# envoy/ksql

Measured on AMD Instinct MI355X. Metric: records/sec, windowed GROUP BY (COUNT(*) TUMBLING 5 s GROUP BY card_number HAVING > 3), higher is better.
Workload: dtype int64

## Files before the change

ksql_amd/csrc/khip_agg_c1.hip:

```cpp
#include <algorithm>
#include <cstdio>
#include <type_traits>
#include <vector>

#include "khip_part.hpp"
#include "khip_sort.hpp"

namespace khip {

constexpr int C1_TILE = 65536;
constexpr int C1_NT = 512;
constexpr int C1_CH = 8192;
template <class T>
__device__ __forceinline__ T c1_ld(const T* p) {
  return *p;
}
constexpr int C1_SEGMAX = 512;
constexpr int C1_SEGB = 7;
constexpr int C1_SEGOF = 512;
constexpr uint32_t C1_SENT = 0x80000000u;

__device__ __forceinline__ int bits_of(uint64_t v) { return v ? 64 - __clzll((long long)v) : 0; }

__device__ __forceinline__ int64_t ci_ld(const int64_t* ci, int k) {
  const uint64_t v = (uint64_t)__hip_atomic_load(&ci[k], __ATOMIC_RELAXED, __HIP_MEMORY_SCOPE_AGENT);
  const uint32_t lo = __builtin_amdgcn_readfirstlane((uint32_t)v), hi = __builtin_amdgcn_readfirstlane((uint32_t)(v >> 32));
  return (int64_t)(((uint64_t)hi << 32) | lo);
}

template <int U, int NT, class R, bool W>
__device__ __forceinline__ uint32_t stage_step_runs(const R (&rec)[U], const uint32_t (&t32)[U], const uint32_t (&bin)[U],
                                                const bool (&ok)[U], int nb, uint32_t* cnt, uint32_t* sbase, int* wsum,
                                                R* sp, uint32_t* lt32, R* __restrict__ out, uint32_t* __restrict__ outT,
                                                int64_t gs, uint32_t* lrc, uint16_t* lro) {
  const int t = threadIdx.x, lane = t & 63, wave = t >> 6;
  uint32_t rank[U];
#pragma unroll
  for (int u = 0; u < U; u++) rank[u] = ok[u] ? atomicAdd(&cnt[bin[u]], 1u) : 0u;
  lds_barrier();
  const uint32_t c = t < nb ? cnt[t] : 0u;
  uint32_t incl = c;
  for (int off = 1; off < 64; off <<= 1) {
    const uint32_t y = __shfl_up(incl, off, 64);
    if (lane >= off) incl += y;
  }
  if (lane == 63) wsum[wave] = (int)incl;
  lds_barrier();
  uint32_t before = 0, tot = 0;
#pragma unroll
  for (int k = 0; k < NT / 64; k++) {
    before += k < wave ? (uint32_t)wsum[k] : 0u;
    tot += (uint32_t)wsum[k];
  }
  if (t < nb) {
    sbase[t] = before + incl - c;
    lrc[t] = c;
    lro[t] = (uint16_t)(before + incl - c);
    cnt[t] = 0u;
  }
  lds_barrier();
#pragma unroll
  for (int u = 0; u < U; u++)
    if (ok[u]) {
      const uint32_t i = sbase[bin[u]] + rank[u];
      sp[i] = rec[u];
      if (W) lt32[i] = t32[u];
    }
  lds_barrier();
  R* o = out + gs * (int64_t)(U * NT);
  for (uint32_t j = t; j < tot; j += NT) o[j] = sp[j];
  if (W) {
    uint32_t* oT = outT + gs * (int64_t)(U * NT);
    for (uint32_t j = t; j < tot; j += NT) oT[j] = lt32[j];
  }
  return tot;
}

template <int NT, class R>
__device__ __forceinline__ void step_krange(const R* sp, uint32_t tot, uint32_t kmask, uint32_t* lkr) {
  uint32_t mn = 0xFFFFFFFFu, mx = 0u;
  for (uint32_t j = threadIdx.x; j < tot; j += NT) {
    uint64_t w;
    if constexpr (sizeof(R) == 16) w = ((const ulonglong2*)sp)[j].x;
    else w = (uint64_t)((const int64_t*)sp)[j];
    const uint32_t kr = (uint32_t)(w >> 32) & kmask;
    mn = kr < mn ? kr : mn;
    mx = kr > mx ? kr : mx;
  }
  for (int off = 32; off > 0; off >>= 1) {
    const uint32_t a = __shfl_xor(mn, off, 64), b = __shfl_xor(mx, off, 64);
    mn = a < mn ? a : mn;
    mx = b > mx ? b : mx;
  }
  if ((threadIdx.x & 63) == 0 && mx >= mn) {
    atomicMin(&lkr[0], mn);
    atomicMax(&lkr[1], mx);
  }
}

__host__ __device__ constexpr size_t run_stage_lds(int nb, int S, int rec_bytes, bool w) {
  return (size_t)nb * 8 + (size_t)S * rec_bytes + (w ? (size_t)S * 4 : 0);
}
__host__ __device__ constexpr size_t run_cnt_lds(int nb, int spt) { return (size_t)nb * spt * 6; }

template <int SPT, int NT>
__device__ __forceinline__ void flush_run_counts(const uint32_t* lrc, const uint16_t* lro, int B, int st_last, int64_t t,
                                                 int64_t nSt, uint32_t* __restrict__ rcnt, uint16_t* __restrict__ roff) {
  static_assert(SPT % 8 == 0, "whole 16-byte stores");
  for (int b = threadIdx.x; b < B; b += NT) {
    uint32_t* rc = rcnt + (int64_t)b * nSt + t * SPT;
    uint16_t* ro = roff + (int64_t)b * nSt + t * SPT;
#pragma unroll
    for (int q = 0; q < SPT / 4; q++) {
      uint32_t v[4];
#pragma unroll
      for (int k = 0; k < 4; k++) v[k] = 4 * q + k <= st_last ? lrc[(4 * q + k) * B + b] : 0u;
      *(uint4*)(rc + 4 * q) = make_uint4(v[0], v[1], v[2], v[3]);
    }
#pragma unroll
    for (int q = 0; q < SPT / 8; q++) {
      uint32_t w[4];
#pragma unroll
      for (int k = 0; k < 4; k++) {
        const int s0 = 8 * q + 2 * k;
        const uint32_t lo = s0 <= st_last ? lro[s0 * B + b] : 0u, hi = s0 + 1 <= st_last ? lro[(s0 + 1) * B + b] : 0u;
        w[k] = lo | hi << 16;
      }
      *(uint4*)(ro + 8 * q) = make_uint4(w[0], w[1], w[2], w[3]);
    }
  }
}

__device__ __forceinline__ void run_bases(const int64_t* __restrict__ keys, const int64_t* __restrict__ ts, int64_t n,
                                          const int64_t* __restrict__ stream_time, int64_t kb_in, int has_kb,
                                          int kfield, int64_t* ci, int64_t* T0, int64_t* kb) {
  const int64_t st0 = *stream_time;
  const int64_t t0 = n > 0 ? ts[0] : 0;
  *T0 = st0 >= 0 ? st0 : (t0 > 0 ? t0 : 0);
  *kb = has_kb ? kb_in : (int64_t)((uint64_t)keys[0] - (1ULL << (kfield - 1)));
  if (blockIdx.x == 0 && threadIdx.x == 0) {
    ci[CI_T0] = *T0;
    ci[CI_KBASE] = *kb;
  }
}

__device__ __forceinline__ void run_krange(const uint32_t* lkr, int kfail, int64_t kb, int64_t* ci) {
  if (lkr[1] >= lkr[0]) {
    atomicMin((long long*)&ci[CI_KMIN], (long long)((uint64_t)kb + lkr[0]));
    atomicMax((long long*)&ci[CI_KMAX], (long long)((uint64_t)kb + lkr[1]));
  }
  if (kfail) atomicOr((unsigned long long*)&ci[CI_KFAIL], 1ULL);
}

template <int U, int NT, bool WIDE, bool ST>
__global__ __launch_bounds__(NT) __attribute__((amdgpu_waves_per_eu(4))) void k_c1_scatter(
    const int64_t* __restrict__ keys, const int64_t* __restrict__ ts, const uint8_t* __restrict__ kv,
    const uint8_t* __restrict__ rv, int64_t n, int64_t nT, int log2B, uint32_t* __restrict__ rcnt,
    uint16_t* __restrict__ roff, int64_t nSt, uint64_t* __restrict__ srec, int64_t* __restrict__ tilestat,
    int64_t* __restrict__ tpart, int64_t* __restrict__ ci, const int64_t* __restrict__ st_at,
    uint32_t* __restrict__ srecT, int64_t size, int64_t adv, FastDiv fd, int64_t grace,
    const int64_t* __restrict__ stream_time, int64_t kb_in, int has_kb) {
  extern __shared__ __attribute__((aligned(16))) char smem[];
  __shared__ int wsum[NT / 64];
  __shared__ unsigned long long lc[4];
  __shared__ int lt[2][2];
  __shared__ int lfail, lkfail;
  __shared__ uint32_t lkr[2];
  constexpr int S = U * NT;
  constexpr int SPT = C1_TILE / S;
  const int B = 1 << log2B;
  const int64_t t = tile_of(blockIdx.x, nT);
  uint32_t* cnt = (uint32_t*)smem;
  uint32_t* sbase = cnt + B;
  int64_t* sp = (int64_t*)(smem + (size_t)B * 8);
  uint32_t* lt32 = (uint32_t*)(sp + S);
  uint32_t* lrc = (uint32_t*)(smem + run_stage_lds(B, S, 8, WIDE));
  uint16_t* lro = (uint16_t*)(lrc + SPT * B);
  for (int b = threadIdx.x; b < B; b += NT) cnt[b] = 0u;
  if (threadIdx.x < 4) lc[threadIdx.x] = 0;
  if (threadIdx.x < 2) {
    lt[threadIdx.x][0] = INT32_MIN;
    lt[threadIdx.x][1] = INT32_MAX;
  }
  if (threadIdx.x == 0) {
    lfail = lkfail = 0;
    lkr[0] = 0xFFFFFFFFu;
    lkr[1] = 0u;
  }
  int64_t T0, kb;
  run_bases(keys, ts, n, stream_time, kb_in, has_kb, 32, ci, &T0, &kb);
  const int shift = log2B == 0 ? 64 : 64 - log2B;
  const uint32_t bmask = (uint32_t)(B - 1);
  const int64_t base = t * C1_TILE;
  const int64_t end = base + C1_TILE < n ? base + C1_TILE : n;
  int c_acc = 0, c_nk = 0, c_nr = 0, c_bt = 0;
  uint32_t kor = 0u;
  int64_t x[U], k[U];
  auto load_step = [&](int64_t i0, int64_t (&dx)[U], int64_t (&dk)[U]) {
#pragma unroll
    for (int u = 0; u < U; u++) {
      int64_t i = i0 + (int64_t)u * NT;
      i = i < end ? i : end - 1;
      dx[u] = ts[i];
      dk[u] = keys[i];
    }
  };
  int64_t t_rmax = -1, t_min = INT64_MAX, t_bound = INT64_MAX;
  bool t_ok = true;
  auto publish = [&](int64_t, int st) {
    const int mx = lt[st & 1][0], mn = lt[st & 1][1];
    if (mx != INT32_MIN) {
      const int64_t smx = T0 + mx, smn = T0 + mn;
      t_rmax = smx > t_rmax ? smx : t_rmax;
      t_min = smn < t_min ? smn : t_min;
      const int64_t fw = first_window_start_fd(smn, size, adv, fd) + size;
      const int64_t b = grace > ((int64_t)1 << 61) ? INT64_MAX : fw + grace - 1;
      t_bound = b < t_bound ? b : t_bound;
      t_ok = t_ok && t_rmax <= b;
    }
    lt[st & 1][0] = INT32_MIN;
    lt[st & 1][1] = INT32_MAX;
  };
  lds_barrier();
  int64_t s0 = base;
  int st_last = -1;
  if (s0 < end) load_step(s0 + threadIdx.x, x, k);
  for (int st = 0; s0 < end; s0 += S, st++) {
    st_last = st;
    const int64_t i0 = s0 + threadIdx.x;
    bool ok[U];
    uint32_t bin[U], t32[U];
    int64_t rec[U];
    int tmx = INT32_MIN, tmn = INT32_MAX;
#pragma unroll
    for (int u = 0; u < U; u++) {
      const int64_t i = i0 + (int64_t)u * NT;
      ok[u] = i < end;
      const bool kok = bit_get(kv, ok[u] ? i : base), rok = bit_get(rv, ok[u] ? i : base);
      const bool valid = ok[u] && kok && rok && x[u] >= 0;
      c_nk += ok[u] && !kok;
      c_nr += ok[u] && kok && !rok;
      c_bt += ok[u] && kok && rok && x[u] < 0;
      c_acc += valid;
      const int64_t sx = ST ? st_at[ok[u] ? i : base] : x[u];
      const int64_t d = x[u] - T0;
      if (valid && (d <= (int64_t)INT32_MIN || d > (int64_t)INT32_MAX)) {
        lfail = 1;
#ifdef KHIP_TUNING
        if (ci[CI_N - 1] == 1 && (threadIdx.x & 63) == 0) printf("[c1 scatter] t %ld i %ld x %ld T0 %ld\n", (long)t, (long)i, (long)x[u], (long)T0);
#endif
      }
      if constexpr (ST) {
        const int64_t ds = sx - T0;
        if (valid && (ds <= (int64_t)INT32_MIN || ds > (int64_t)INT32_MAX)) lfail = 1;
        tmx = valid && (int)ds > tmx ? (int)ds : tmx;
      } else {
        tmx = valid && (int)d > tmx ? (int)d : tmx;
      }
      tmn = valid && (int)d < tmn ? (int)d : tmn;
      const uint64_t hk = key_hash(k[u]);
      bin[u] = stage_bin(hk, shift, bmask);
      t32[u] = valid ? (uint32_t)d : C1_SENT;
      const uint64_t kd = (uint64_t)k[u] - (uint64_t)kb;
      if (!WIDE) kor |= ok[u] ? (uint32_t)(kd >> 32) : 0u;
      rec[u] = WIDE ? (int64_t)hk : (int64_t)((kd << 32) | (uint64_t)t32[u]);
    }
    if (s0 + S < end) load_step(i0 + S, x, k);
    const uint32_t tot = stage_step_runs<U, NT, int64_t, WIDE>(rec, t32, bin, ok, B, cnt, sbase, wsum, sp, lt32,
                                                               (int64_t*)srec, srecT, t * SPT + st, lrc + st * B,
                                                               lro + st * B);
    if (!WIDE) step_krange<NT, int64_t>(sp, tot, 0xFFFFFFFFu, lkr);
    for (int off = 32; off > 0; off >>= 1) {
      const int a = __shfl_xor(tmx, off, 64), b = __shfl_xor(tmn, off, 64);
      tmx = a > tmx ? a : tmx;
      tmn = b < tmn ? b : tmn;
    }
    if ((threadIdx.x & 63) == 0 && tmx != INT32_MIN) {
      atomicMax(&lt[st & 1][0], tmx);
      atomicMin(&lt[st & 1][1], tmn);
    }
    if (threadIdx.x == 0 && st > 0) publish(s0 - S, st - 1);
  }
  flush_run_counts<SPT, NT>(lrc, lro, B, st_last, t, nSt, rcnt, roff);
  if (!WIDE && kor) lkfail = 1;
  __syncthreads();
  if (threadIdx.x == 0 && s0 > base) publish(s0 - S, st_last);
  if (!WIDE && threadIdx.x == 0) run_krange(lkr, lkfail, kb, ci);
  c_acc = wave_sum(c_acc);
  c_nk = wave_sum(c_nk);
  c_nr = wave_sum(c_nr);
  c_bt = wave_sum(c_bt);
  if ((threadIdx.x & 63) == 0) {
    if (c_acc) atomicAdd(&lc[0], (unsigned long long)c_acc);
    if (c_nk) atomicAdd(&lc[1], (unsigned long long)c_nk);
    if (c_nr) atomicAdd(&lc[2], (unsigned long long)c_nr);
    if (c_bt) atomicAdd(&lc[3], (unsigned long long)c_bt);
  }
  __syncthreads();
  if (threadIdx.x == 0) {
    int64_t* tp = tpart + t * T_NPART;
    tp[T_ACCEPTED] = (int64_t)lc[0];
    tp[T_NULL_KEY] = (int64_t)lc[1];
    tp[T_NULL_ROW] = (int64_t)lc[2];
    tp[T_BAD_TS] = (int64_t)lc[3];
    tp[T_APPLIED] = (int64_t)lc[0];
    tp[T_LATE] = 0;
    if (lfail) atomicOr((unsigned long long*)&ci[CI_TFAIL], 1ULL);
    int64_t* ts4 = tilestat + t * 4;
    ts4[0] = t_rmax;
    ts4[1] = t_min;
    ts4[2] = t_bound;
    ts4[3] = t_ok ? 1 : 0;
  }
}

__global__ __launch_bounds__(256) void k_c1_krange(const int64_t* __restrict__ keys, int64_t stride, int64_t n,
                                                   long long* __restrict__ out) {
  int64_t mx = INT64_MIN, mxn = INT64_MIN;
  for (int64_t i = blockIdx.x * (int64_t)blockDim.x + threadIdx.x; i < n; i += (int64_t)gridDim.x * blockDim.x) {
    const int64_t k = keys[i * stride];
    mx = k > mx ? k : mx;
    mxn = ~k > mxn ? ~k : mxn;
  }
  for (int off = 32; off > 0; off >>= 1) {
    const int64_t a = __shfl_xor(mx, off, 64), b = __shfl_xor(mxn, off, 64);
    mx = a > mx ? a : mx;
    mxn = b > mxn ? b : mxn;
  }
  if ((threadIdx.x & 63) == 0) {
    atomicMax(&out[0], (long long)mxn);
    atomicMax(&out[1], (long long)mx);
  }
}

__global__ __launch_bounds__(256) void k_c1_bases(const uint32_t* __restrict__ rpos, int64_t nSt, int B,
                                                  int64_t* __restrict__ bb) {
  for (int b = threadIdx.x; b <= B; b += blockDim.x) bb[b] = (int64_t)rpos[(int64_t)b * nSt];
}

__global__ __launch_bounds__(256) void k_c1_chunks(const int* __restrict__ cstart, int B, const int64_t* __restrict__ bb,
                                                   const uint32_t* __restrict__ rpos, int64_t nSt, int ch,
                                                   const int64_t* __restrict__ ci, uint32_t* __restrict__ cinfo) {
  if (ci_ld(ci, CI_GATE) == 0) return;
  const int w = blockIdx.x * blockDim.x + threadIdx.x;
  if (w >= (int)ci_ld(ci, CI_NCHUNK)) return;
  int a = 0, e = B;
  while (e - a > 1) {
    const int m = (a + e) >> 1;
    if (cstart[m] <= w) a = m;
    else e = m;
  }
  const int b = a;
  const int64_t lo = bb[b] + (int64_t)(w - cstart[b]) * ch;
  const int64_t len = bb[b + 1] - lo < ch ? bb[b + 1] - lo : ch;
  const uint32_t* rp = rpos + (int64_t)b * nSt;
  int64_t sa = 0, se = nSt;
  while (se - sa > 1) {
    const int64_t m = (sa + se) >> 1;
    if ((int64_t)rp[m] <= lo) sa = m;
    else se = m;
  }
  int64_t ta = sa, te = nSt;
  while (te - ta > 1) {
    const int64_t m = (ta + te) >> 1;
    if ((int64_t)rp[m] < lo + len) ta = m;
    else te = m;
  }
  cinfo[2 * w] = (uint32_t)sa;
  cinfo[2 * w + 1] = (uint32_t)(te - sa);
}

__device__ __forceinline__ void chunk_map(const uint32_t* __restrict__ rp, const uint16_t* __restrict__ ro,
                                          const uint32_t* __restrict__ cinfo, int w, int64_t S, int64_t lo, int len,
                                          uint32_t* map) {
  const int64_t s0 = cinfo[2 * w];
  const int R = (int)cinfo[2 * w + 1];
  for (int k = threadIdx.x; k < R; k += blockDim.x) {
    const int64_t s = s0 + k, p = (int64_t)rp[s], pe = (int64_t)rp[s + 1];
    const int64_t a = p > lo ? p : lo, e = pe < lo + len ? pe : lo + len;
    const uint32_t src = (uint32_t)(s * S + (int64_t)ro[s] + (a - p));
    for (int64_t x = a; x < e; x++) map[x - lo] = src + (uint32_t)(x - a);
  }
  __syncthreads();
}

__global__ __launch_bounds__(1024) void k_c1_check(
    const int64_t* __restrict__ tilestat, int64_t nT, int64_t size, int64_t adv, FastDiv fd, int64_t grace,
    int64_t close0, int fresh, int log2B, int log2P, int wide, int ch, int kbmax, int pbits,
    const int64_t* __restrict__ bb, int* __restrict__ cstart,
    int64_t* __restrict__ ci, int64_t* __restrict__ stream_time, int64_t* __restrict__ res,
    unsigned long long* __restrict__ ctr, unsigned long long* __restrict__ closed_ctr, unsigned long long closed_n) {
  __shared__ int64_t wmx[16];
  __shared__ int64_t red[4][16];
  __shared__ int lslow;
  __shared__ int lnch[512 + 1];
  const int lane = threadIdx.x & 63, wave = threadIdx.x >> 6;
  if (threadIdx.x == 0) lslow = 0;
  const int64_t st0 = *stream_time;
  const int64_t K = (nT + 1023) / 1024;
  const int64_t g0 = threadIdx.x * K, g1 = g0 + K < nT ? g0 + K : nT;
  int64_t m = -1;
  for (int64_t g = g0; g < g1; g++) m = tilestat[4 * g] > m ? tilestat[4 * g] : m;
  const int64_t incl = wave_incl_max(m);
  if (lane == 63) wmx[wave] = incl;
  __syncthreads();
  int64_t pre = st0;
  for (int w = 0; w < wave; w++) pre = wmx[w] > pre ? wmx[w] : pre;
  const int64_t excl = __shfl_up(incl, 1, 64);
  int64_t run = lane == 0 ? pre : (excl > pre ? excl : pre);
  int64_t gmn = INT64_MAX, gmx = -1;
  bool slow = false;
  for (int64_t g = g0; g < g1; g++) {
    const int64_t* t4 = tilestat + 4 * g;
    const int64_t mx = t4[0], mn = t4[1];
    if (mn != INT64_MAX) {
      slow |= t4[3] == 0 || run > t4[2];
      gmn = mn < gmn ? mn : gmn;
    }
    run = mx > run ? mx : run;
    gmx = mx > gmx ? mx : gmx;
  }
  if (slow) lslow = 1;
  for (int off = 32; off > 0; off >>= 1) {
    const int64_t a = __shfl_xor(gmn, off, 64), b = __shfl_xor(gmx, off, 64);
    gmn = a < gmn ? a : gmn;
    gmx = b > gmx ? b : gmx;
  }
  if (lane == 0) {
    red[0][wave] = gmn;
    red[1][wave] = gmx;
  }
  const int B = 1 << log2B;
  for (int b = threadIdx.x; b < B; b += 1024) lnch[b] = (int)((bb[b + 1] - bb[b] + ch - 1) / ch);
  __syncthreads();
  if (threadIdx.x) return;
  for (int w = 0; w < 16; w++) {
    gmn = red[0][w] < gmn ? red[0][w] : gmn;
    gmx = red[1][w] > gmx ? red[1][w] : gmx;
  }
  int acc = 0, mxc = 0;
  for (int b = 0; b < B; b++) {
    cstart[b] = acc;
    acc += lnch[b];
    mxc = lnch[b] > mxc ? lnch[b] : mxc;
  }
  cstart[B] = acc;
  const int64_t kmin = ci_ld(ci, CI_KMIN), kmax = ci_ld(ci, CI_KMAX);
  const bool tfail = ci_ld(ci, CI_TFAIL) != 0, kfail = ci_ld(ci, CI_KFAIL) != 0;
  ci[CI_KMIN] = INT64_MAX;
  ci[CI_KMAX] = INT64_MIN;
  ci[CI_TFAIL] = 0;
  ci[CI_KFAIL] = 0;
  bool ok = !lslow && !tfail && mxc <= C1_SEGMAX && (wide || kmax >= kmin);
#ifdef KHIP_TUNING
  if (ci[CI_N - 1] == 1)
    printf("[c1 check] tfail %d slow %d mxc %d kmin %ld kmax %ld gmn %ld gmx %ld T0 %ld st0 %ld nT %ld\n", (int)tfail,
           (int)lslow, mxc, (long)kmin, (long)kmax, (long)gmn, (long)gmx, (long)ci[CI_T0], (long)st0, (long)nT);
#endif
  const uint64_t krange = kmax >= kmin ? (uint64_t)kmax - (uint64_t)kmin : 0;
  const bool fits = !wide && !kfail && krange < ((1ULL << kbmax) - 1);
  const int64_t kb = ci_ld(ci, CI_KBASE);
  ci[CI_FITS] = fits ? 1 : 0;
  ci[CI_REASON] = ok && !wide && kfail ? 2 : (ok && !wide && !fits ? 1 : 0);
  ci[CI_KMINC] = kmin;
  ci[CI_KSHIFT] = (int64_t)((uint64_t)kmin - (uint64_t)kb);
  ok = ok && (wide || fits);
  int64_t lo = INT64_MAX, hi = INT64_MIN;
  if (gmx >= 0) {
    const int64_t l = gmn - size + adv;
    lo = (int64_t)fast_udiv((uint64_t)(l > 0 ? l : 0), fd);
    hi = (int64_t)fast_udiv((uint64_t)gmx, fd);
  }
  if (!fresh) {
    int64_t rlo = res[0];
    const int64_t rhi = res[1];
    if (close0 != INT64_MIN && rlo != INT64_MAX) {
      const int64_t c = close0 - size;
      const int64_t lb = c >= 0 ? (int64_t)fast_udiv((uint64_t)c, fd) + 1 : 0;
      rlo = rlo > lb ? rlo : lb;
    }
    lo = rlo < lo ? rlo : lo;
    hi = rhi > hi ? rhi : hi;
  }
  const bool none = lo > hi;
  if (none) lo = hi = 0;
  ok = ok && (uint64_t)(hi - lo) < (wide ? ((uint64_t)1 << log2P) - 1 : (pbits ? 0x7FFFFFFEull : 0xFFFFFFFEull));
  const int wbits = bits_of((uint64_t)(hi - lo)), kbits = bits_of(krange);
  ci[CI_GATE] = ok ? 1 : 0;
  if (!ok) return;
  ci[CI_WBASE] = lo;
  ci[CI_WHI] = hi - lo;
  ci[CI_WBITS] = wbits;
  ci[CI_KBITS] = kbits;
  ci[CI_KRANGE] = (int64_t)krange;
  ci[CI_ID32] = !wide && kbits + wbits + pbits <= 31 ? 1 : 0;
  ci[CI_WIDE] = wide;
  ci[CI_TMIN] = gmx >= 0 ? gmn : 0;
  ci[CI_TMAX] = gmx;
  ci[CI_NCHUNK] = acc;
  *stream_time = gmx > st0 ? gmx : st0;
  res[0] = none ? INT64_MAX : lo;
  res[1] = none ? INT64_MIN : hi;
  ctr[CTR_ADDED] = ctr[CTR_FAILED] = ctr[CTR_NEED] = 0ULL;
  if (closed_ctr) *closed_ctr = closed_n;
}

template <int U, int NT, bool WIDE>
__global__ __launch_bounds__(NT) __attribute__((amdgpu_waves_per_eu(4))) void k_c1_refine(
    const uint64_t* __restrict__ srcA, const int64_t* __restrict__ bb, const int* __restrict__ cstart, int log2B,
    int log2P, int fbits, uint64_t* __restrict__ srec, uint16_t* __restrict__ seg, const int64_t* __restrict__ ci,
    const uint32_t* __restrict__ srcAT, uint32_t* __restrict__ srecT, const uint32_t* __restrict__ rpos,
    const uint16_t* __restrict__ roff, int64_t nSt, int64_t S, const uint32_t* __restrict__ cinfo) {
  if (ci_ld(ci, CI_GATE) == 0) return;
  const int w = blockIdx.x;
  if (w >= (int)ci_ld(ci, CI_NCHUNK)) return;
  extern __shared__ __attribute__((aligned(16))) char smem[];
  __shared__ int lb, lnv;
  __shared__ int wsum[NT / 64];
  static_assert(U * NT == C1_CH, "refine chunk");
  const int F = 1 << fbits, B = 1 << log2B;
  uint32_t* cnt = (uint32_t*)smem;
  uint32_t* sbase = cnt + F;
  uint64_t* stage = (uint64_t*)(smem + (size_t)F * 8);
  for (int f = threadIdx.x; f < F; f += NT) cnt[f] = 0u;
  if (threadIdx.x == 0) lb = -1;
  __syncthreads();
  for (int b = threadIdx.x; b < B; b += NT)
    if (cstart[b] <= w && w < cstart[b + 1]) lb = b;
  __syncthreads();
  const int b = lb;
  if (b < 0) return;
  const int64_t lo = bb[b] + (int64_t)(w - cstart[b]) * C1_CH;
  const int64_t bend = bb[b + 1];
  const int len = (int)(bend - lo < C1_CH ? bend - lo : C1_CH);
  const int64_t kmin = ci_ld(ci, CI_KMINC);
  const uint64_t kshift = WIDE ? 0 : (uint64_t)ci_ld(ci, CI_KSHIFT) << 32;
  const int shift = 64 - log2P;
  const uint32_t* rp = rpos + (int64_t)b * nSt;
  const uint16_t* ro = roff + (int64_t)b * nSt;
  chunk_map(rp, ro, cinfo, w, S, lo, len, (uint32_t*)stage);
  uint64_t r[U];
  uint32_t f[U], rank[U], t32[U];
#pragma unroll
  for (int u = 0; u < U; u++) {
    const int j = threadIdx.x + u * NT;
    const uint32_t src = ((const uint32_t*)stage)[j < len ? j : len - 1];
    r[u] = c1_ld(srcA + src) - kshift;
    if constexpr (WIDE) t32[u] = c1_ld(srcAT + src);
  }
#pragma unroll
  for (int u = 0; u < U; u++) {
    const int j = threadIdx.x + u * NT;
    const bool v = j < len && (WIDE ? t32[u] : (uint32_t)r[u]) != C1_SENT;
    f[u] = WIDE ? (uint32_t)(r[u] >> shift) & (uint32_t)(F - 1)
                : (uint32_t)(key_hash(kmin + (int64_t)(r[u] >> 32)) >> shift) & (uint32_t)(F - 1);
    rank[u] = v ? atomicAdd(&cnt[f[u]], 1u) : 0xFFFFFFFFu;
  }
  __syncthreads();
  {
    const int t = threadIdx.x, lane = t & 63, wave = t >> 6;
    const uint32_t c = t < F ? cnt[t] : 0u;
    uint32_t incl = c;
    for (int off = 1; off < 64; off <<= 1) {
      const uint32_t y = __shfl_up(incl, off, 64);
      if (lane >= off) incl += y;
    }
    if (lane == 63) wsum[wave] = (int)incl;
    __syncthreads();
    uint32_t before = 0, tot = 0;
#pragma unroll
    for (int k = 0; k < NT / 64; k++) {
      before += k < wave ? (uint32_t)wsum[k] : 0u;
      tot += (uint32_t)wsum[k];
    }
    if (t < F) {
      sbase[t] = before + incl - c;
      seg[(int64_t)w * (F + 1) + t] = (uint16_t)(before + incl - c);
    }
    if (t == 0) {
      seg[(int64_t)w * (F + 1) + F] = (uint16_t)tot;
      lnv = (int)tot;
    }
  }
  __syncthreads();
  const int nv = lnv;
#pragma unroll
  for (int u = 0; u < U; u++)
    if (rank[u] != 0xFFFFFFFFu) stage[sbase[f[u]] + rank[u]] = r[u];
  __syncthreads();
  for (int j = threadIdx.x; j < nv; j += NT) srec[lo + j] = stage[j];
  if constexpr (WIDE) {
    __syncthreads();
    uint32_t* stage32 = (uint32_t*)stage;
#pragma unroll
    for (int u = 0; u < U; u++)
      if (rank[u] != 0xFFFFFFFFu) stage32[sbase[f[u]] + rank[u]] = t32[u];
    __syncthreads();
    for (int j = threadIdx.x; j < nv; j += NT) srecT[lo + j] = stage32[j];
  }
}

#ifdef KHIP_TUNING
#define C1M_T(k)                                                                        \
  do {                                                                                  \
    if (dbg && threadIdx.x == 0) {                                                      \
      const unsigned long long now_ = wall_clock64();                                   \
      atomicAdd(&dbg[(k)], now_ - t_last);                                              \
      t_last = now_;                                                                    \
    }                                                                                   \
  } while (0)
#define C1M_T0 unsigned long long t_last = dbg ? wall_clock64() : 0ULL
#else
#define C1M_T(k) \
  do {           \
  } while (0)
#define C1M_T0 (void)dbg
#endif

struct C1Q {
  int32_t log2P, fbits, log2H, sw, hv_active, hv_op, hmax;
  int64_t size, adv, cmax, hv_i64;
  FastDiv fd;
  FastDiv32 fd32;
// ... 596 lines not shown
          c += ct[e];
        }
        *(longlong2*)dst = make_longlong2((int64_t)row[0], (int64_t)row[1]);
        *(longlong2*)(dst + 2) = make_longlong2((int64_t)w2, (int64_t)c);
        const bool now = !q.hv_active || c1q_having(q, c);
        nh += q.hv_active && now ? 1 : 0;
        if (q.chg)
          q.chg[(uint64_t)p * q.cmax + ri] =
              e >= 0 ? (uint8_t)(CHG_TOUCHED | (!q.hv_active || c1q_having(q, row[3]) ? CHG_OLD : 0) | (now ? CHG_NEW : 0))
                     : (uint8_t)0;
      }
      cur += __popcll(bl);
    }
    if (nrow > 0) lds_barrier();
    const uint32_t wmask = wbits ? (1u << wbits) - 1u : 0u;
    for (int k = lb0; k < lb1; k += 64) {
      const int i = k + lane;
      const uint32_t e = i < lb1 ? list[i] : dummy;
      const uint32_t rv = rt[e];
      const bool used = i < lb1;
      const bool isnew = used && !(rv & RT_MATCHED);
      const uint64_t bl = __ballot(isnew);
      if (isnew) {
        const uint64_t ri = cur + __popcll(bl & lt);
        uint64_t* dst = dst0 + ri * q.sw;
        const ID id = ids[e];
        int64_t key, wi;
        if constexpr (WIDE) {
          wi = (int64_t)((uint64_t)id & (((uint64_t)1 << q.log2P) - 1));
          key = key_of_hash(((uint64_t)p << (64 - q.log2P)) | ((uint64_t)id >> q.log2P));
        } else if constexpr (sizeof(ID) == 4) {
          key = kmin + (int64_t)((uint32_t)id >> wbits);
          wi = (int64_t)((uint32_t)id & wmask);
        } else {
          key = kmin + (int64_t)((uint64_t)id >> 32);
          wi = (int64_t)((uint64_t)id & 0xFFFFFFFFull);
        }
        const uint32_t c = ct[e];
        *(longlong2*)dst = make_longlong2(key, (wbase + wi) * q.adv);
        *(longlong2*)(dst + 2) = make_longlong2(tmin + (int64_t)rv - 1, (int64_t)c);
        const bool now = !q.hv_active || c1q_having(q, c);
        nh += q.hv_active && now ? 1 : 0;
        if (q.chg) q.chg[(uint64_t)p * q.cmax + ri] = (uint8_t)(CHG_TOUCHED | (now ? CHG_NEW : 0));
      }
      if (used) {
        ids[e] = EMPTY;
        rt[e] = 0u;
        ct[e] = 0u;
      }
      cur += __popcll(bl);
    }
    if (q.hv_active) {
      nh = (int)wave_sum(nh);
      nhc = (int)wave_sum(nhc);
      if (lane == 0 && nh) atomicAdd(&hnew[p], (unsigned long long)nh);
      if (lane == 0 && nhc) atomicAdd(hclosed, (unsigned long long)nhc);
    }
    lds_barrier();
    C1M_T(4);
    if (threadIdx.x == 0) nnew = 0;
    lds_barrier();
  }
}

constexpr int C1V_CH = 4096;
constexpr int C1V_MAXW = 8;

typedef uint64_t c1v_u2 __attribute__((ext_vector_type(2)));
__device__ __forceinline__ ulonglong2 ld_nt2(const ulonglong2* p) {
  const c1v_u2 v = c1_ld((const c1v_u2*)p);
  return make_ulonglong2(v.x, v.y);
}

struct C1VCol {
  const void* data;
  const uint8_t* valid;
  int32_t type;
};


template <int U, int NT, bool ST, bool ROWS>
__global__ __launch_bounds__(NT) __attribute__((amdgpu_waves_per_eu(4))) void k_c1v_scatter(
    const int64_t* __restrict__ keys, const int64_t* __restrict__ ts, const uint8_t* __restrict__ kv,
    const uint8_t* __restrict__ rv, C1VCol vc, RowsIn ri, int64_t n, int64_t nT, int log2B, uint32_t* __restrict__ rcnt,
    uint16_t* __restrict__ roff, int64_t nSt, ulonglong2* __restrict__ srec, int64_t* __restrict__ tilestat,
    int64_t* __restrict__ tpart, int64_t* __restrict__ ci, const int64_t* __restrict__ st_at, int64_t size, int64_t adv,
    FastDiv fd, int hop, int64_t grace, const int64_t* __restrict__ stream_time, int64_t kb_in, int has_kb) {
  extern __shared__ __attribute__((aligned(16))) char smem[];
  __shared__ int wsum[NT / 64];
  __shared__ unsigned long long lc[5];
  __shared__ int lt[2][2];
  __shared__ int lfail, lkfail;
  __shared__ uint32_t lkr[2];
  constexpr int S = U * NT;
  constexpr int SPT = C1_TILE / S;
  const int B = 1 << log2B;
  const int64_t t = tile_of(blockIdx.x, nT);
  uint32_t* cnt = (uint32_t*)smem;
  uint32_t* sbase = cnt + B;
  ulonglong2* sp = (ulonglong2*)(smem + (size_t)B * 8);
  uint32_t* lrc = (uint32_t*)(smem + run_stage_lds(B, S, 16, false));
  uint16_t* lro = (uint16_t*)(lrc + SPT * B);
  for (int b = threadIdx.x; b < B; b += NT) cnt[b] = 0u;
  if (threadIdx.x < 5) lc[threadIdx.x] = 0;
  if (threadIdx.x < 2) {
    lt[threadIdx.x][0] = INT32_MIN;
    lt[threadIdx.x][1] = INT32_MAX;
  }
  if (threadIdx.x == 0) {
    lfail = lkfail = 0;
    lkr[0] = 0xFFFFFFFFu;
    lkr[1] = 0u;
  }
  int64_t T0, kb;
  if constexpr (ROWS) run_bases((const int64_t*)ri.rows, (const int64_t*)ri.rows + 1, n, stream_time, kb_in, has_kb, 31, ci, &T0, &kb);
  else run_bases(keys, ts, n, stream_time, kb_in, has_kb, 31, ci, &T0, &kb);
  const int shift = log2B == 0 ? 64 : 64 - log2B;
  const uint32_t bmask = (uint32_t)(B - 1);
  const int64_t base = t * C1_TILE;
  const int64_t end = base + C1_TILE < n ? base + C1_TILE : n;
  int c_acc = 0, c_nk = 0, c_nr = 0, c_bt = 0, c_app = 0;
  uint32_t kor = 0u;
  int64_t x[U], k[U], v[U];
  uint32_t vm[ROWS ? U : 1];
  int64_t rst[ROWS && ST ? U : 1];
  auto load_step = [&](int64_t i0) {
#pragma unroll
    for (int u = 0; u < U; u++) {
      int64_t i = i0 + (int64_t)u * NT;
      i = i < end ? i : end - 1;
      if constexpr (ROWS) {
        const uint64_t* r = ri.rows + i * (int64_t)ri.rw;
        if (ri.rw == 4 && ri.vword == 2) {
          const ulonglong2 a = ((const ulonglong2*)r)[0], b = ((const ulonglong2*)r)[1];
          k[u] = (int64_t)a.x;
          x[u] = (int64_t)a.y;
          v[u] = (int64_t)b.x;
          vm[u] = (uint32_t)b.y;
        } else {
          k[u] = (int64_t)r[0];
          x[u] = (int64_t)r[1];
          v[u] = (int64_t)r[ri.vword];
          vm[u] = (uint32_t)r[ri.rw - 1];
        }
        if constexpr (ST) rst[u] = (int64_t)r[ri.rw - 2];
      } else {
        x[u] = ts[i];
        k[u] = keys[i];
        v[u] = vc.type == KHIP_TYPE_INT32 ? (int64_t)((const int32_t*)vc.data)[i] : ((const int64_t*)vc.data)[i];
      }
    }
  };
  int64_t t_rmax = -1, t_min = INT64_MAX, t_bound = INT64_MAX;
  bool t_ok = true;
  auto publish = [&](int64_t, int st) {
    const int mx = lt[st & 1][0], mn = lt[st & 1][1];
    if (mx != INT32_MIN) {
      const int64_t smx = T0 + mx, smn = T0 + mn;
      t_rmax = smx > t_rmax ? smx : t_rmax;
      t_min = smn < t_min ? smn : t_min;
      const int64_t fw = first_window_start_fd(smn, size, adv, fd) + size;
      const int64_t b = grace > ((int64_t)1 << 61) ? INT64_MAX : fw + grace - 1;
      t_bound = b < t_bound ? b : t_bound;
      t_ok = t_ok && t_rmax <= b;
    }
    lt[st & 1][0] = INT32_MIN;
    lt[st & 1][1] = INT32_MAX;
  };
  lds_barrier();
  int64_t s0 = base;
  int st_last = -1;
  if (s0 < end) load_step(s0 + threadIdx.x);
  for (int st = 0; s0 < end; s0 += S, st++) {
    st_last = st;
    const int64_t i0 = s0 + threadIdx.x;
    bool ok[U];
    uint32_t bin[U];
    ulonglong2 rec[U];
    int tmx = INT32_MIN, tmn = INT32_MAX;
#pragma unroll
    for (int u = 0; u < U; u++) {
      const int64_t i = i0 + (int64_t)u * NT;
      ok[u] = i < end;
      const int64_t ii = ok[u] ? i : base;
      const bool kok = ROWS || bit_get(kv, ii), rok = ROWS || bit_get(rv, ii);
      const bool vok = ROWS ? ((vm[ROWS ? u : 0] >> ri.vbit) & 1u) != 0 : bit_get(vc.valid, ii);
      const bool valid = ok[u] && kok && rok && x[u] >= 0;
      c_nk += ok[u] && !kok;
      c_nr += ok[u] && kok && !rok;
      c_bt += ok[u] && kok && rok && x[u] < 0;
      c_acc += valid;
      const int64_t d = x[u] - T0;
      if (valid && (d <= (int64_t)INT32_MIN || d > (int64_t)INT32_MAX)) {
        lfail = 1;
#ifdef KHIP_TUNING
        if (ci[CI_N - 1] == 1 && (threadIdx.x & 63) == 0) printf("[c1 scatter] t %ld i %ld x %ld T0 %ld\n", (long)t, (long)i, (long)x[u], (long)T0);
#endif
      }
      if constexpr (ST) {
        const int64_t ds = (ROWS ? rst[ROWS ? u : 0] : st_at[ii]) - T0;
        if (valid && (ds <= (int64_t)INT32_MIN || ds > (int64_t)INT32_MAX)) lfail = 1;
        tmx = valid && (int)ds > tmx ? (int)ds : tmx;
      } else {
        tmx = valid && (int)d > tmx ? (int)d : tmx;
      }
      tmn = valid && (int)d < tmn ? (int)d : tmn;
      if (hop && valid) {
        const int64_t lo = x[u] - size + adv;
        c_app += (int)((int64_t)fast_udiv((uint64_t)x[u], fd) - (int64_t)fast_udiv((uint64_t)(lo > 0 ? lo : 0), fd) + 1);
      }
      bin[u] = stage_bin(key_hash(k[u]), shift, bmask);
      const uint64_t kd = (uint64_t)k[u] - (uint64_t)kb;
      kor |= ok[u] ? (uint32_t)(kd >> 31) : 0u;
      const uint64_t w0 = ((kd & 0x7FFFFFFFull) << 32) | (uint64_t)(valid ? (uint32_t)d : C1_SENT);
      rec[u] = make_ulonglong2(w0 | (vok ? (1ULL << 63) : 0ULL), (uint64_t)v[u]);
    }
    if (s0 + S < end) load_step(i0 + S);
    uint32_t t32u[U];
    const uint32_t tot = stage_step_runs<U, NT, ulonglong2, false>(rec, t32u, bin, ok, B, cnt, sbase, wsum, sp, nullptr,
                                                                   srec, nullptr, t * SPT + st, lrc + st * B,
                                                                   lro + st * B);
    step_krange<NT, ulonglong2>(sp, tot, 0x7FFFFFFFu, lkr);
    for (int off = 32; off > 0; off >>= 1) {
      const int a = __shfl_xor(tmx, off, 64), b = __shfl_xor(tmn, off, 64);
      tmx = a > tmx ? a : tmx;
      tmn = b < tmn ? b : tmn;
    }
    if ((threadIdx.x & 63) == 0 && tmx != INT32_MIN) {
      atomicMax(&lt[st & 1][0], tmx);
      atomicMin(&lt[st & 1][1], tmn);
    }
    if (threadIdx.x == 0 && st > 0) publish(s0 - S, st - 1);
  }
  flush_run_counts<SPT, NT>(lrc, lro, B, st_last, t, nSt, rcnt, roff);
  if (kor) lkfail = 1;
  __syncthreads();
  if (threadIdx.x == 0 && s0 > base) publish(s0 - S, st_last);
  if (threadIdx.x == 0) run_krange(lkr, lkfail, kb, ci);
  c_acc = wave_sum(c_acc);
  c_nk = wave_sum(c_nk);
  c_nr = wave_sum(c_nr);
  c_bt = wave_sum(c_bt);
  c_app = wave_sum(c_app);
  if ((threadIdx.x & 63) == 0) {
    if (c_acc) atomicAdd(&lc[0], (unsigned long long)c_acc);
    if (c_nk) atomicAdd(&lc[1], (unsigned long long)c_nk);
    if (c_nr) atomicAdd(&lc[2], (unsigned long long)c_nr);
    if (c_bt) atomicAdd(&lc[3], (unsigned long long)c_bt);
    if (c_app) atomicAdd(&lc[4], (unsigned long long)c_app);
  }
  __syncthreads();
  if (threadIdx.x == 0) {
    int64_t* tp = tpart + t * T_NPART;
    tp[T_ACCEPTED] = (int64_t)lc[0];
    tp[T_NULL_KEY] = (int64_t)lc[1];
    tp[T_NULL_ROW] = (int64_t)lc[2];
    tp[T_BAD_TS] = (int64_t)lc[3];
    tp[T_APPLIED] = hop ? (int64_t)lc[4] : (int64_t)lc[0];
    tp[T_LATE] = 0;
    if (lfail) atomicOr((unsigned long long*)&ci[CI_TFAIL], 1ULL);
    int64_t* ts4 = tilestat + t * 4;
    ts4[0] = t_rmax;
    ts4[1] = t_min;
    ts4[2] = t_bound;
    ts4[3] = t_ok ? 1 : 0;
  }
}

template <int U, int NT>
__global__ __launch_bounds__(NT) __attribute__((amdgpu_waves_per_eu(4))) void k_c1v_refine(
    const ulonglong2* __restrict__ srcA, const int64_t* __restrict__ bb, const int* __restrict__ cstart, int log2B,
    int log2P, int fbits, ulonglong2* __restrict__ srec, uint16_t* __restrict__ seg, const int64_t* __restrict__ ci,
    const uint32_t* __restrict__ rpos, const uint16_t* __restrict__ roff, int64_t nSt, int64_t S,
    const uint32_t* __restrict__ cinfo) {
  if (ci_ld(ci, CI_GATE) == 0) return;
  const int w = blockIdx.x;
  if (w >= (int)ci_ld(ci, CI_NCHUNK)) return;
  extern __shared__ __attribute__((aligned(16))) char smem[];
  __shared__ int lb, lnv;
  __shared__ int wsum[NT / 64];
  constexpr int CH = U * NT;
  static_assert(CH == C1V_CH, "refine chunk");
  const int F = 1 << fbits, B = 1 << log2B;
  uint32_t* cnt = (uint32_t*)smem;
  uint32_t* sbase = cnt + F;
  ulonglong2* stage = (ulonglong2*)(smem + (((size_t)F * 8 + 15) & ~(size_t)15));
  for (int f = threadIdx.x; f < F; f += NT) cnt[f] = 0u;
  if (threadIdx.x == 0) lb = -1;
  __syncthreads();
  for (int b = threadIdx.x; b < B; b += NT)
    if (cstart[b] <= w && w < cstart[b + 1]) lb = b;
  __syncthreads();
  const int b = lb;
  if (b < 0) return;
  const int64_t lo = bb[b] + (int64_t)(w - cstart[b]) * CH;
  const int64_t bend = bb[b + 1];
  const int len = (int)(bend - lo < CH ? bend - lo : CH);
  const int64_t kmin = ci_ld(ci, CI_KMINC);
  const uint64_t kshift = (uint64_t)ci_ld(ci, CI_KSHIFT) << 32;
  const int shift = 64 - log2P;
  const uint32_t* rp = rpos + (int64_t)b * nSt;
  const uint16_t* ro = roff + (int64_t)b * nSt;
  chunk_map(rp, ro, cinfo, w, S, lo, len, (uint32_t*)stage);
  ulonglong2 r[U];
  uint32_t f[U], rank[U];
#pragma unroll
  for (int u = 0; u < U; u++) {
    const int j = threadIdx.x + u * NT;
    const uint32_t src = ((const uint32_t*)stage)[j < len ? j : len - 1];
    r[u] = ld_nt2(srcA + src);
    r[u].x -= kshift;
  }
#pragma unroll
  for (int u = 0; u < U; u++) {
    const int j = threadIdx.x + u * NT;
    const bool v = j < len && (uint32_t)r[u].x != C1_SENT;
    f[u] = (uint32_t)(key_hash(kmin + (int64_t)((r[u].x >> 32) & 0x7FFFFFFFull)) >> shift) & (uint32_t)(F - 1);
    rank[u] = v ? atomicAdd(&cnt[f[u]], 1u) : 0xFFFFFFFFu;
  }
  __syncthreads();
  {
    const int t = threadIdx.x, lane = t & 63, wave = t >> 6;
    const uint32_t c = t < F ? cnt[t] : 0u;
    uint32_t incl = c;
    for (int off = 1; off < 64; off <<= 1) {
      const uint32_t y = __shfl_up(incl, off, 64);
      if (lane >= off) incl += y;
    }
    if (lane == 63) wsum[wave] = (int)incl;
    __syncthreads();
    uint32_t before = 0, tot = 0;
#pragma unroll
    for (int k = 0; k < NT / 64; k++) {
      before += k < wave ? (uint32_t)wsum[k] : 0u;
      tot += (uint32_t)wsum[k];
    }
    if (t < F) {
      sbase[t] = before + incl - c;
      seg[(int64_t)w * (F + 1) + t] = (uint16_t)(before + incl - c);
    }
    if (t == 0) {
      seg[(int64_t)w * (F + 1) + F] = (uint16_t)tot;
      lnv = (int)tot;
    }
  }
  __syncthreads();
  const int nv = lnv;
#pragma unroll
  for (int u = 0; u < U; u++)
    if (rank[u] != 0xFFFFFFFFu) stage[sbase[f[u]] + rank[u]] = r[u];
  __syncthreads();
  for (int j = threadIdx.x; j < nv; j += NT) srec[lo + j] = stage[j];
}

struct C1VQ {
  int32_t log2P, fbits, log2H, sw, hmax, f64, fan;
  int32_t off_sum, off_min, off_max, off_rt, off_star, off_cnt, off_list, off_spre;
  int32_t word_op[C1V_MAXW];
  int64_t size, adv, cmax;
  FastDiv fd;
  FastDiv32 fd32;
  uint64_t init[C1V_MAXW];
  HavingDev having;
  uint8_t* chg;
};

template <class T>
__device__ __forceinline__ KLDS T* c1v_plane(char* smem, int off) {
  return (KLDS T*)((KLDS char*)smem + off);
}

constexpr int PM_STAR = 1, PM_CNT = 2, PM_SUM = 4, PM_MIN = 8, PM_MAX = 16, PM_F64 = 32, PM_SPEC = 64;
constexpr int PM_C5 = PM_SPEC | PM_SUM;
constexpr int PM_C3 = PM_SPEC | PM_CNT | PM_SUM | PM_MIN | PM_MAX | PM_F64;
template <int PM>
struct C1VP {
  const C1VQ& q;
  __device__ __forceinline__ bool star() const { return PM ? (PM & PM_STAR) != 0 : q.off_star >= 0; }
  __device__ __forceinline__ bool cnt() const { return PM ? (PM & PM_CNT) != 0 : q.off_cnt >= 0; }
  __device__ __forceinline__ bool sum() const { return PM ? (PM & PM_SUM) != 0 : q.off_sum >= 0; }
  __device__ __forceinline__ bool mn() const { return PM ? (PM & PM_MIN) != 0 : q.off_min >= 0; }
  __device__ __forceinline__ bool mx() const { return PM ? (PM & PM_MAX) != 0 : q.off_max >= 0; }
  __device__ __forceinline__ bool f64() const { return PM ? (PM & PM_F64) != 0 : q.f64 != 0; }
};

template <int PM>
// ... 707 lines not shown
                    s.rw == 2;
  return cnt1 && a->windowed && a->desc.window_kind == KHIP_WINDOW_TUMBLING && s.log2P >= 11 && s.log2P <= 16 &&
         s.mH >= 256 && a->desc.advance_ms <= ((int64_t)1 << 31) && !(a->desc.flags & KHIP_FLAG_PART_CLAIM) &&
         n > 0 && n < ((int64_t)1 << 31) && knob("KHIP_C1P", 1) != 0 && knob("KHIP_PAD", 0) == 0 &&
         knob("KHIP_MERGE", 1) != 0 && knob("KHIP_SCATTER2", 1) != 0;
}

bool c1v_eligible(khip_agg* a, int64_t n, int* col) {
  PartState& s = a->part;
  if (!a->windowed || a->sw > C1V_MAXW || a->ap.n_ops < 1 || s.rw < 2) return false;
  const int64_t size = a->desc.size_ms, adv = a->desc.advance_ms;
  if (a->desc.window_kind == KHIP_WINDOW_HOPPING) {
    if (size % adv != 0 || size / adv > 16) return false;
  } else if (a->desc.window_kind != KHIP_WINDOW_TUMBLING) {
    return false;
  }
  int c = -1, seen = 0;
  for (int o = 0; o < a->ap.n_ops; o++) {
    const UpdOp op = a->ap.ops[o];
    if (op.kind < OP_INC || op.kind > OP_MAX || op.word < 3 || op.word >= a->sw) return false;
    const int bit = op.kind == OP_ADD_F64 ? (1 << OP_ADD_I64) : (1 << op.kind);
    if (seen & bit) return false;
    seen |= bit;
    if (op.kind == OP_INC) continue;
    if (c >= 0 && op.col != c) return false;
    c = op.col;
  }
  if (c < 0) return false;
  const int t = a->ap.col_type[c];
  if (t != KHIP_TYPE_INT32 && t != KHIP_TYPE_INT64 && t != KHIP_TYPE_DOUBLE) return false;
  *col = c;
  return s.log2P >= 11 && s.log2P <= 16 && s.mH >= 256 && adv <= ((int64_t)1 << 31) &&
         !(a->desc.flags & KHIP_FLAG_PART_CLAIM) && n > 0 && n < ((int64_t)1 << 31) && knob("KHIP_C1V", 1) != 0 &&
         knob("KHIP_PAD", 0) == 0 && knob("KHIP_MERGE", 1) != 0 && knob("KHIP_SCATTER2", 1) != 0;
}

constexpr size_t C1V_LDS2 = 80 * 1024 - 256;

static size_t c1v_layout(khip_agg* a, int log2H, int idw, int log2B, C1VQ* q) {
  const size_t E = ((size_t)1 << log2H) + 64, H = (size_t)1 << log2H, B = (size_t)1 << log2B;
  size_t off = E * idw;
  off = (off + 7) & ~(size_t)7;
  q->off_sum = q->off_min = q->off_max = q->off_star = q->off_cnt = -1;
  for (int o = 0; o < a->ap.n_ops; o++) {
    const int k = a->ap.ops[o].kind;
    if (k == OP_ADD_I64 || k == OP_ADD_F64) q->off_sum = 1;
    if (k == OP_MIN) q->off_min = 1;
    if (k == OP_MAX) q->off_max = 1;
    if (k == OP_INC) q->off_star = 1;
    if (k == OP_INC_VALID) q->off_cnt = 1;
  }
  auto place = [&](int32_t* f, size_t bytes) {
    if (*f < 0) return;
    *f = (int32_t)off;
    off += E * bytes;
  };
  place(&q->off_sum, 8);
  place(&q->off_min, 8);
  place(&q->off_max, 8);
  q->off_rt = (int32_t)off;
  off += E * 4;
  place(&q->off_star, 4);
  place(&q->off_cnt, 4);
  off = (off + 15) & ~(size_t)15;
  q->off_list = (int32_t)off;
  off += (H * 2 + 15) & ~(size_t)15;
  q->off_spre = (int32_t)off;
  off += (C1_SEGMAX + 4) * 8 + C1_SEGOF * 2;
  (void)B;
  return off;
}

constexpr int C1V_UV = 4;

struct C1Geo {
  bool val, panes, wide;
  int P, CH, fbits, log2B, B, F;
  int64_t n, nT, S, nSt, nchunk_max;
  size_t seg_bytes;
  int64_t* ci;
  int* cstart;
  uint16_t* seg;
  uint32_t *srecAT, *srecT;
  uint32_t *rc, *rp;
  uint16_t* ro;
  int64_t adv, close0;
  FastDiv fd;
};

struct C1Merge {
  C1Q cq;
  C1VQ vq0;
  int log2H, v_log2H;
  int v_pm;
  int v_wpc;
};

enum C1Next { C1_DONE, C1_DECLINED, C1_AGAIN_KBASE, C1_AGAIN_WIDE };

static khip_status c1_prepare(khip_agg* a, int64_t n, const C1In& in, C1Geo* g) {
  PartState& s = a->part;
  g->val = in.cols != nullptr || in.rows != nullptr;
  g->panes = g->val && a->desc.window_kind == KHIP_WINDOW_HOPPING;
  g->CH = g->val ? C1V_CH : C1_CH;
  g->P = (int)s.P;
  g->fbits = s.log2P - s.log2P / 2;
  g->log2B = s.log2P - g->fbits;
  g->B = 1 << g->log2B;
  g->F = 1 << g->fbits;
  g->n = n;
  g->nT = ceil_div(n, C1_TILE);
  g->S = g->val ? (int64_t)C1V_UV * C1_NT : (int64_t)8 * C1_NT;
  g->nSt = g->nT * (C1_TILE / g->S);
  g->nchunk_max = ceil_div(n, g->CH) + g->B;
  const int64_t B = g->B, nSt = g->nSt, nT = g->nT;
  KHIP_TRY(s.c1rc.ensure((size_t)B * nSt * 4));
  KHIP_TRY(s.c1rp.ensure(((size_t)B * nSt + 1) * 4));
  KHIP_TRY(s.c1ro.ensure((size_t)B * nSt * 2));
  KHIP_TRY(s.c1bb.ensure((size_t)(B + 1) * 8));
  g->seg_bytes = ((size_t)g->nchunk_max * (g->F + 1) * 2 + 255) & ~(size_t)255;
  KHIP_TRY(s.c1seg.ensure(g->seg_bytes + (size_t)(B + 1) * 4));
  KHIP_TRY(s.tilemax.ensure(nT * 32));
  KHIP_TRY(s.tpart.ensure(nT * 8 * T_NPART));
  KHIP_TRY(s.prn.ensure((size_t)g->P * 4));
  KHIP_TRY(s.res.ensure(16));
  KHIP_TRY(s.closed_ctr.ensure(8));
  if (s.scat_cap < n) {
    KHIP_TRY(s.srec.ensure((size_t)(n + 1) * s.rw * 8));
    s.scat_cap = n;
  }
  KHIP_TRY(s.srec.ensure((size_t)(n + 1) * 16));
  KHIP_TRY(s.srecA.ensure((size_t)(n + 1) * std::max(s.rw, 2) * 8));
  if (!s.c1info.p) {
    KHIP_TRY(s.c1info.ensure(CI_N * 8));
    int64_t init[CI_N] = {};
    init[CI_KMIN] = INT64_MAX;
    init[CI_KMAX] = INT64_MIN;
    KHIP_TRY_HIP(hipMemcpy(s.c1info.p, init, sizeof(init), hipMemcpyHostToDevice));
  }
  g->ci = s.c1info.as<int64_t>();
#ifdef KHIP_TUNING
  {
    const int64_t dbg = knob("KHIP_C1_DEBUG", 0);
    KHIP_TRY_HIP(hipMemcpyAsync(g->ci + CI_N - 1, &dbg, 8, hipMemcpyHostToDevice, a->stream));
    KHIP_TRY_HIP(hipStreamSynchronize(a->stream));
  }
#endif
  g->cstart = (int*)(s.c1seg.as<char>() + g->seg_bytes);
  g->seg = s.c1seg.as<uint16_t>();
  g->adv = a->desc.advance_ms;
  g->fd = make_fastdiv(g->adv);
  g->close0 = a->host_stream_time >= 0 ? a->host_stream_time - a->grace : INT64_MIN;
  g->wide = !g->val && s.c1_wide;
  g->srecAT = (uint32_t*)(s.srecA.as<uint64_t>() + n + 1);
  g->srecT = (uint32_t*)(s.srec.as<uint64_t>() + n + 1);
  g->rc = s.c1rc.as<uint32_t>();
  g->rp = s.c1rp.as<uint32_t>();
  g->ro = s.c1ro.as<uint16_t>();
  return KHIP_OK;
}

static khip_status c1_scatter(khip_agg* a, const C1In& in, const C1Geo& g) {
  PartState& s = a->part;
  ev_record_part(a, 0);
  const int has_kb = s.c1_kb_valid ? 1 : 0;
  const int64_t* st_at = in.st_at;
  if (g.val) {
    constexpr int UV = C1V_UV;
    const RowsIn* rows = in.rows;
    const C1VCol vc{rows ? nullptr : in.cols->data[in.vcol], rows ? nullptr : in.cols->valid[in.vcol],
                    a->ap.col_type[in.vcol]};
    const RowsIn ri = rows ? *rows : RowsIn{};
    auto sk = rows ? (st_at ? k_c1v_scatter<UV, C1_NT, true, true> : k_c1v_scatter<UV, C1_NT, false, true>)
                   : (st_at ? k_c1v_scatter<UV, C1_NT, true, false> : k_c1v_scatter<UV, C1_NT, false, false>);
    const size_t lds = run_stage_lds(g.B, UV * C1_NT, 16, false) + run_cnt_lds(g.B, C1_TILE / (UV * C1_NT));
    if (lds > 64 * 1024) hipFuncSetAttribute((const void*)sk, hipFuncAttributeMaxDynamicSharedMemorySize, (int)lds);
    hipLaunchKernelGGL(sk, dim3(g.nT), dim3(C1_NT), lds, a->stream, in.keys, in.ts, in.kv, in.rv, vc, ri, g.n, g.nT,
                       g.log2B, g.rc, g.ro, g.nSt, (ulonglong2*)s.srecA.p, s.tilemax.as<int64_t>(),
                       s.tpart.as<int64_t>(), g.ci, st_at, a->desc.size_ms, g.adv, g.fd,
                       a->desc.size_ms != g.adv ? 1 : 0, a->grace, (const int64_t*)a->stream_time.as<int64_t>(),
                       s.c1_kbase, has_kb);
  } else {
    constexpr int U = 8;
    auto sk = g.wide ? (st_at ? k_c1_scatter<U, C1_NT, true, true> : k_c1_scatter<U, C1_NT, true, false>)
                     : (st_at ? k_c1_scatter<U, C1_NT, false, true> : k_c1_scatter<U, C1_NT, false, false>);
    const size_t lds = run_stage_lds(g.B, U * C1_NT, 8, g.wide) + run_cnt_lds(g.B, C1_TILE / (U * C1_NT));
    if (lds > 64 * 1024) hipFuncSetAttribute((const void*)sk, hipFuncAttributeMaxDynamicSharedMemorySize, (int)lds);
    hipLaunchKernelGGL(sk, dim3(g.nT), dim3(C1_NT), lds, a->stream, in.keys, in.ts, in.kv, in.rv, g.n, g.nT, g.log2B,
                       g.rc, g.ro, g.nSt, s.srecA.as<uint64_t>(), s.tilemax.as<int64_t>(), s.tpart.as<int64_t>(), g.ci,
                       st_at, g.srecAT, a->desc.size_ms, g.adv, g.fd, a->grace,
                       (const int64_t*)a->stream_time.as<int64_t>(), s.c1_kbase, has_kb);
  }
  KHIP_TRY_HIP(hipGetLastError());
  KHIP_TRY((ksort::scan_excl<uint32_t, uint32_t>(a->stream, s.c1scan, g.rc, g.rp, (int64_t)g.B * g.nSt, true, nullptr)));
  hipLaunchKernelGGL(k_c1_bases, dim3(1), dim3(256), 0, a->stream, (const uint32_t*)g.rp, g.nSt, g.B,
                     s.c1bb.as<int64_t>());
  ev_record_part(a, 1);
  return KHIP_OK;
}

static khip_status c1_refine(khip_agg* a, const C1Geo& g) {
  PartState& s = a->part;
  if (g.val) {
    auto rk = k_c1v_refine<C1V_CH / C1_NT, C1_NT>;
    const size_t lds = (((size_t)g.F * 8 + 15) & ~(size_t)15) + (size_t)C1V_CH * 16;
    hipFuncSetAttribute((const void*)rk, hipFuncAttributeMaxDynamicSharedMemorySize, (int)lds);
    hipLaunchKernelGGL(rk, dim3((unsigned)g.nchunk_max), dim3(C1_NT), lds, a->stream, (const ulonglong2*)s.srecA.p,
                       s.c1bb.as<int64_t>(), g.cstart, g.log2B, s.log2P, g.fbits, (ulonglong2*)s.srec.p, g.seg, g.ci,
                       (const uint32_t*)g.rp, (const uint16_t*)g.ro, g.nSt, g.S,
                       (const uint32_t*)s.c1ci.as<uint32_t>());
  } else {
    constexpr int U = C1_CH / C1_NT;
    auto rk = g.wide ? k_c1_refine<U, C1_NT, true> : k_c1_refine<U, C1_NT, false>;
    const size_t lds = (size_t)g.F * 8 + (size_t)C1_CH * 8;
    if (lds > 64 * 1024) hipFuncSetAttribute((const void*)rk, hipFuncAttributeMaxDynamicSharedMemorySize, (int)lds);
    hipLaunchKernelGGL(rk, dim3((unsigned)g.nchunk_max), dim3(C1_NT), lds, a->stream, s.srecA.as<uint64_t>(),
                       s.c1bb.as<int64_t>(), g.cstart, g.log2B, s.log2P, g.fbits, s.srec.as<uint64_t>(), g.seg, g.ci,
                       (const uint32_t*)g.srecAT, g.srecT, (const uint32_t*)g.rp, (const uint16_t*)g.ro, g.nSt, g.S,
                       (const uint32_t*)s.c1ci.as<uint32_t>());
  }
  KHIP_TRY_HIP(hipGetLastError());
  return KHIP_OK;
}

static khip_status c1_records(khip_agg* a, const C1In& in, const C1Geo& g) {
  PartState& s = a->part;
  KHIP_TRY(c1_scatter(a, in, g));
  hipLaunchKernelGGL(k_c1_check, dim3(1), dim3(1024), 0, a->stream, s.tilemax.as<int64_t>(), g.nT, a->desc.size_ms,
                     g.adv, g.fd, a->grace, g.close0, s.res_fresh ? 1 : 0, g.log2B, s.log2P, g.wide ? 1 : 0, g.CH,
                     g.val ? 31 : 32, g.panes ? 1 : 0, s.c1bb.as<int64_t>(), g.cstart, g.ci,
                     a->stream_time.as<int64_t>(), s.res.as<int64_t>(), s.ctr.as<unsigned long long>(),
                     s.closed_ctr.as<unsigned long long>(), (unsigned long long)s.closed_n);
  KHIP_TRY(s.c1ci.ensure((size_t)g.nchunk_max * 8));
  hipLaunchKernelGGL(k_c1_chunks, dim3((unsigned)ceil_div(g.nchunk_max, 256)), dim3(256), 0, a->stream,
                     (const int*)g.cstart, g.B, (const int64_t*)s.c1bb.as<int64_t>(), (const uint32_t*)g.rp, g.nSt, g.CH,
                     (const int64_t*)g.ci, s.c1ci.as<uint32_t>());
  KHIP_TRY(c1_refine(a, g));
  ev_record_part(a, 2);
  return KHIP_OK;
}

static C1Q c1_make_q(khip_agg* a, const C1Geo& g, int log2H) {
  C1Q cq{};
  cq.log2P = a->part.log2P;
  cq.fbits = g.fbits;
  cq.log2H = log2H;
  cq.sw = a->sw;
  cq.hv_active = a->having.active;
  cq.hv_op = a->having.op;
  cq.hv_i64 = a->having.i64;
  cq.hmax = (int)((int64_t)(1 << log2H) * 3 / 4);
  cq.size = a->desc.size_ms;
  cq.adv = g.adv;
  cq.fd = g.fd;
  cq.fd32 = make_fastdiv32((uint32_t)g.adv);
  return cq;
}

static void c1v_make_q(khip_agg* a, const C1Geo& g, int vcol, C1Merge* m) {
  C1VQ& vq0 = m->vq0;
  m->v_log2H = 12;
  while (m->v_log2H > 9 && c1v_layout(a, m->v_log2H, 4, g.log2B, &vq0) > C1V_LDS2) m->v_log2H--;
  m->v_log2H = (int)knob("KHIP_C1V_LOG2H", m->v_log2H);

  vq0.log2P = a->part.log2P;
  vq0.fbits = g.fbits;
  vq0.log2H = m->v_log2H;
  vq0.sw = a->sw;
  vq0.hmax = (int)((int64_t)(1 << m->v_log2H) * 3 / 4);
  vq0.fan = (int)(a->desc.size_ms / g.adv);
  vq0.f64 = 0;
  for (int k = 0; k < C1V_MAXW; k++) {
    vq0.word_op[k] = -1;
    vq0.init[k] = (uint64_t)a->init.w[k];
  }
  for (int o = 0; o < a->ap.n_ops; o++) {
    vq0.word_op[a->ap.ops[o].word] = a->ap.ops[o].kind;
    if (a->ap.ops[o].kind == OP_ADD_F64) vq0.f64 = 1;
  }
  if (a->ap.col_type[vcol] == KHIP_TYPE_DOUBLE) vq0.f64 = 1;
  int pm = 0;
  for (int o = 0; o < a->ap.n_ops; o++) {
    const int k = a->ap.ops[o].kind;
    pm |= k == OP_INC ? PM_STAR : k == OP_INC_VALID ? PM_CNT : k == OP_MIN ? PM_MIN : k == OP_MAX ? PM_MAX : PM_SUM;
  }
  pm |= PM_SPEC | (vq0.f64 ? PM_F64 : 0);
  m->v_pm = ((pm != PM_C5 && pm != PM_C3) || knob("KHIP_C1V_SPEC", 1) == 0) ? 0 : pm;
  vq0.size = a->desc.size_ms;
  vq0.adv = g.adv;
  vq0.fd = g.fd;
  vq0.fd32 = make_fastdiv32((uint32_t)g.adv);
  vq0.having = a->having;
}

static khip_status c1_launch_merge(khip_agg* a, const C1Geo& g, const C1Merge& m, int pass, const uint32_t* wk,
                                   int64_t nwork, unsigned long long* dbg) {
  PartState& s = a->part;
  unsigned long long* ctr = s.ctr.as<unsigned long long>();
  uint8_t* chg = a->changelog ? a->chg.as<uint8_t>() : nullptr;
  for (int idw = g.wide ? 1 : 0; idw < 2 && g.val; idw++) {
    C1VQ vq = m.vq0;
    const size_t lds = c1v_layout(a, m.v_log2H, idw == 0 ? 4 : 8, g.log2B, &vq);
    vq.cmax = s.cmax;
    vq.chg = chg;
    auto pick = [&](auto pmc) {
      constexpr int PMv = decltype(pmc)::value;
      return g.panes ? (idw == 0 ? k_c1v_merge<512, 2, uint32_t, true, 4, PMv> : k_c1v_merge<512, 2, uint64_t, true, 4, PMv>)
                     : (idw == 0 ? k_c1v_merge<512, 2, uint32_t, false, 4, PMv> : k_c1v_merge<512, 2, uint64_t, false, 4, PMv>);
    };
    auto mk = m.v_pm == PM_C5 ? pick(std::integral_constant<int, PM_C5>{})
                              : (m.v_pm == PM_C3 ? pick(std::integral_constant<int, PM_C3>{}) : pick(std::integral_constant<int, 0>{}));
    hipFuncSetAttribute((const void*)mk, hipFuncAttributeMaxDynamicSharedMemorySize, (int)lds);
    KHIP_TRY(s.c1vq.ensure(sizeof(C1VQ)));
    KHIP_TRY(s.c1vq_h.ensure(2 * sizeof(C1VQ)));
    C1VQ* hq = (C1VQ*)s.c1vq_h.p + idw;
    *hq = vq;
    KHIP_TRY_HIP(hipMemcpyAsync(s.c1vq.p, hq, sizeof(C1VQ), hipMemcpyHostToDevice, a->stream));
    const int64_t vgrid = std::min<int64_t>(nwork, (int64_t)s.n_cu * (lds <= C1V_LDS2 ? m.v_wpc : 1));
    hipLaunchKernelGGL(mk, dim3(vgrid), dim3(512), lds, a->stream, s.c1vq.as<C1VQ>(), wk, nwork, s.c1bb.as<int64_t>(),
                       g.cstart, g.seg, (const ulonglong2*)s.srec.p, pass == 0 ? 1 : 0, s.buf[0].as<uint64_t>(),
                       s.buf[1].as<uint64_t>(), s.sel.as<uint8_t>(), s.cnt.as<int64_t>(),
                       s.newcnt.as<unsigned long long>(), s.fail.as<uint8_t>(), ctr + CTR_NEED, g.close0,
                       s.closed.as<uint64_t>(), s.closed_ctr.as<unsigned long long>(),
                       (unsigned long long)s.closed_cap, g.ci, s.hnew.as<unsigned long long>(), ctr + CTR_HAVING_CLOSED,
                       s.prn.as<uint32_t>(), dbg);
  }
  C1Q cq = m.cq;
  cq.cmax = s.cmax;
  cq.chg = chg;
  const int64_t grid = std::min<int64_t>(nwork, (int64_t)s.n_cu * knob("KHIP_MERGE_WG_PER_CU", 2));
  for (int idw = g.wide ? 1 : 0; idw < 2 && !g.val; idw++) {
    auto mk = g.wide ? k_c1_merge<512, 3, uint64_t, true>
                     : (idw == 0 ? k_c1_merge<512, 4, uint32_t, false> : k_c1_merge<512, 4, uint64_t, false>);
    const size_t lds = c1_merge_lds(m.log2H, idw == 0 ? 4 : 8, g.log2B);
    hipFuncSetAttribute((const void*)mk, hipFuncAttributeMaxDynamicSharedMemorySize, (int)lds);
    hipLaunchKernelGGL(mk, dim3(grid), dim3(512), lds, a->stream, cq, wk, nwork, s.c1bb.as<int64_t>(), g.cstart, g.seg,
                       s.srec.as<uint64_t>(), pass == 0 ? 1 : 0, s.buf[0].as<uint64_t>(), s.buf[1].as<uint64_t>(),
                       s.sel.as<uint8_t>(), s.cnt.as<int64_t>(), s.newcnt.as<unsigned long long>(),
                       s.fail.as<uint8_t>(), ctr + CTR_NEED, g.close0, s.closed.as<uint64_t>(),
                       s.closed_ctr.as<unsigned long long>(), (unsigned long long)s.closed_cap, g.ci,
                       s.hnew.as<unsigned long long>(), ctr + CTR_HAVING_CLOSED, s.prn.as<uint32_t>(),
                       (const uint32_t*)g.srecT, dbg);
  }
  KHIP_TRY_HIP(hipGetLastError());
  return KHIP_OK;
}

static khip_status c1_declined_next(khip_agg* a, const C1In& in, const C1Geo& g, bool kretried, C1Next* next) {
  PartState& s = a->part;
  const int64_t* hci = s.info()->c1info;
  bool go_wide = !g.val && hci[CI_REASON] == 1;
  if (hci[CI_REASON] == 2 && !kretried) {
    long long kr[2] = {INT64_MIN, INT64_MIN};
    KHIP_TRY(s.c1scan.ensure(16));
    KHIP_TRY_HIP(hipMemcpyAsync(s.c1scan.p, kr, 16, hipMemcpyHostToDevice, a->stream));
    hipLaunchKernelGGL(k_c1_krange, dim3((unsigned)std::min<int64_t>(ceil_div(g.n, 256), 2048)), dim3(256), 0,
                       a->stream, in.rows ? (const int64_t*)in.rows->rows : in.keys,
                       in.rows ? (int64_t)in.rows->rw : 1, g.n, s.c1scan.as<long long>());
    KHIP_TRY_HIP(hipMemcpyAsync(kr, s.c1scan.p, 16, hipMemcpyDeviceToHost, a->stream));
    KHIP_TRY_HIP(hipStreamSynchronize(a->stream));
    const int64_t kmin = (int64_t)~(uint64_t)kr[0], kmax = (int64_t)kr[1];
    if ((uint64_t)kmax - (uint64_t)kmin < (1ULL << (g.val ? 31 : 32)) - 1) {
      s.c1_kbase = kmin;
      s.c1_kb_valid = true;
      *next = C1_AGAIN_KBASE;
      return KHIP_OK;
    }
    go_wide = !g.val;
  }
  if (go_wide) s.c1_wide = true;
  *next = go_wide ? C1_AGAIN_WIDE : C1_DECLINED;
  return KHIP_OK;
}

static void c1_start_bits(PartState& s, int64_t hm) {
  if ((int64_t)s.c1psbits.size() == s.P && s.c1ps_hmax == hm) return;
  int s0 = 0;
  while (s0 < RETRY_MAX_SBITS && s.hint_groups / s.P > (hm * 7 / 10) << s0) s0++;
  s.c1psbits.assign(s.P, (uint8_t)s0);
  s.c1ps_hmax = hm;
}

khip_status c1_push(khip_agg* a, int64_t n, const C1In& in, int64_t* tot, bool* declined) {
  PartState& s = a->part;
  *declined = false;
  const bool probe = knob("KHIP_AGG_PROBE", 0) != 0;
  bool kretried = false, wide_tried = false;
  for (;;) {
    C1Geo g;
    KHIP_TRY(c1_prepare(a, n, in, &g));
    KHIP_TRY(part_grow_closed(a));
    KHIP_TRY(c1_records(a, in, g));
    C1Merge m{};
    m.log2H = (int)knob("KHIP_C1_LOG2H", 12);
    m.cq = c1_make_q(a, g, m.log2H);
    m.v_wpc = (int)knob("KHIP_C1V_WG_PER_CU", 2);
    if (g.val) c1v_make_q(a, g, in.vcol, &m);
    c1_start_bits(s, g.val ? m.vq0.hmax : m.cq.hmax);
    RetryPlan r;
    retry_begin(r, s.c1psbits);
    const bool subs0 = !r.work.empty();
    if (subs0) KHIP_TRY(part_upload_plan(a, r.image));
    std::vector<uint8_t> host_fail;
    DevBuf dbgbuf;
    if (probe) {
      KHIP_TRY(dbgbuf.ensure(64));
      KHIP_TRY_HIP(hipMemsetAsync(dbgbuf.p, 0, 64, a->stream));
    }
    PushInfo* pi = s.info();
    const unsigned long long* c2 = pi->ctr;
    int64_t added_total = 0;
    C1Next next = C1_DONE;
    for (int pass = 0;; pass++) {
      unsigned long long* dbg = probe && pass == 0 ? dbgbuf.as<unsigned long long>() : nullptr;
      if (pass > 0) KHIP_TRY_HIP(hipMemsetAsync(s.ctr.p, 0, CTR_PER_PASS * 8, a->stream));
      const uint32_t* wk = (pass == 0 && !subs0) ? nullptr : s.work.as<uint32_t>();
      const int64_t nwork = wk ? (int64_t)r.work.size() : g.P;
      KHIP_TRY(c1_launch_merge(a, g, m, pass, wk, nwork, dbg));
      KHIP_TRY(part_pass_commit(a, pass, r, pass == 0 ? (const int64_t*)g.ci : (const int64_t*)nullptr,
                                s.prn.as<uint32_t>(), s.closed_ctr.as<unsigned long long>(), g.nT));
      if (pass == 0) KHIP_TRY_HIP(hipMemcpyAsync(pi->c1info, g.ci, CI_N * 8, hipMemcpyDeviceToHost, a->stream));
      KHIP_TRY_HIP(hipMemcpyAsync(&pi->closed_n, s.closed_ctr.p, 8, hipMemcpyDeviceToHost, a->stream));
      KHIP_TRY_HIP(hipStreamSynchronize(a->stream));
      if (pass == 0 && pi->c1info[CI_GATE] == 0) {
        KHIP_TRY(c1_declined_next(a, in, g, kretried, &next));
        break;
      }
      if (pass == 0 && g.wide && ++s.c1_wide_n % 64 == 0) s.c1_wide = false;
      if (pass == 0 && !g.wide) {
        const int64_t km = pi->c1info[CI_KMINC], slack = (int64_t)1 << (g.val ? 26 : 28);
        s.c1_kbase = km >= INT64_MIN + slack ? km - slack : km;
        s.c1_kb_valid = true;
      }
      if (dbg) {
        unsigned long long ph[8] = {};
        if (hipMemcpy(ph, dbgbuf.p, sizeof(ph), hipMemcpyDeviceToHost) == hipSuccess) {
          const double us = (double)std::min<int64_t>(g.P, 2 * s.n_cu) * 100.0;
          fprintf(stderr, "[%s merge probe] per workgroup (us): start+evict %.1f records %.1f fold %.1f "
                  "mark+count+reserve %.1f write %.1f\n", g.val ? "c1v" : "c1", ph[0] / us, ph[1] / us, ph[2] / us,
                  ph[3] / us, ph[4] / us);
        }
      }
      if (c2[CTR_NEED] & C1_FATAL)
        return fail(KHIP_E_DEVICE, "the closed store's capacity would be exceeded by a merge's closed rows");
      added_total += (int64_t)c2[CTR_ADDED];
      KHIP_TRY(part_pass_failed(a, &host_fail));
#ifdef KHIP_TUNING
      if (knob("KHIP_C1_TRACE", 0) != 0) {
        int64_t nsub, ft, fr;
        part_retry_trace_counts(r, wk != nullptr, host_fail, &nsub, &ft, &fr);
        fprintf(stderr,
                "[c1 trace] val=%d P=%d cmax=%lld log2H=%d pass=%d items=%lld sub_items=%lld failed=%llu fail_table=%lld "
                "fail_region=%lld closed_before=%lld closed_after=%llu\n",
                g.val ? 1 : 0, g.P, (long long)s.cmax, g.val ? m.v_log2H : m.log2H, pass, (long long)nwork,
                (long long)nsub, c2[CTR_FAILED], (long long)ft, (long long)fr, (long long)s.closed_n, pi->closed_n);
      }
#endif
      if (c2[CTR_FAILED] == 0) break;
      KHIP_TRY(part_plan_retry(a, r, pass, host_fail));
    }
    if (next == C1_AGAIN_KBASE) {
      kretried = true;
      continue;
    }
    if (next == C1_AGAIN_WIDE && !wide_tried) {
      wide_tried = true;
      kretried = false;
      continue;
    }
    if (next != C1_DONE) {
      *declined = true;
      return KHIP_OK;
    }
    retry_learn(s.c1psbits, r);
    s.res_fresh = false;
    s.last_c1 = true;
    part_push_epilogue(a, (int64_t)pi->closed_n, added_total, tot);
    return KHIP_OK;
  }
}

}
```

ksql_amd/csrc/khip_agg_internal.hpp:

```cpp
#pragma once

#include <vector>

#include "khip_dict.hpp"
#include "khip_util.hpp"

namespace khip {

constexpr int BLOCK = 256;
constexpr int ITEMS = 8;
constexpr int RPB = BLOCK * ITEMS;
constexpr int MAX_COLS = 8;
constexpr int MAX_OPS = 40;
constexpr int MAX_PROBE = 2048;
constexpr int MAX_FANOUT = 4095;
constexpr int64_t EMPTY_WS = INT64_MIN;
constexpr int NPART = 8;

enum { P_ACCEPTED, P_NULL_KEY, P_NULL_ROW, P_BAD_TS, P_APPLIED, P_LATE, P_FAILED, P_NEW };

enum OpKind : int8_t {
  OP_INC = 0, OP_INC_VALID, OP_ADD_I64, OP_ADD_F64, OP_MIN, OP_MAX, OP_TOPK, OP_TOPK_DISTINCT, OP_ADD_HI32, OP_ADD_SQ,
  OP_PAIR_N, OP_PAIR_SUM, OP_PAIR_SQ, OP_PAIR_XY
};
// ... 433 lines not shown
  if (result_is_double(h.a)) {
    if (dv != dv) return h.op == KHIP_OP_NE;
    c = dv < h.f64 ? -1 : (dv > h.f64 ? 1 : 0);
  } else {
    c = iv < h.i64 ? -1 : (iv > h.i64 ? 1 : 0);
  }
  switch (h.op) {
    case KHIP_OP_GT: return c > 0;
    case KHIP_OP_GE: return c >= 0;
    case KHIP_OP_LT: return c < 0;
    case KHIP_OP_LE: return c <= 0;
    case KHIP_OP_EQ: return c == 0;
    case KHIP_OP_NE: return c != 0;
  }
  return false;
}

__device__ __forceinline__ bool having_only(const uint64_t* s, const HavingDev& h) {
  if (!h.active) return true;
  int64_t iv = 0;
  double dv = 0.0;
  if (!decode_result(s, h.a, &iv, &dv)) return false;
  int c;
  if (result_is_double(h.a)) {
    if (dv != dv) return h.op == KHIP_OP_NE;
    c = dv < h.f64 ? -1 : (dv > h.f64 ? 1 : 0);
  } else {
    c = iv < h.i64 ? -1 : (iv > h.i64 ? 1 : 0);
  }
  switch (h.op) {
    case KHIP_OP_GT: return c > 0;
    case KHIP_OP_GE: return c >= 0;
    case KHIP_OP_LT: return c < 0;
    case KHIP_OP_LE: return c <= 0;
    case KHIP_OP_EQ: return c == 0;
    case KHIP_OP_NE: return c != 0;
  }
  return false;
}

__device__ __forceinline__ bool having_ok(const uint64_t* s, const HavingDev& h) {
  if (!pull_ok(s, h)) return false;
  if (!h.active) return true;
  int64_t iv = 0;
  double dv = 0.0;
  if (!decode_result(s, h.a, &iv, &dv)) return false;
  int c;
  if (result_is_double(h.a)) {
    if (dv != dv) return h.op == KHIP_OP_NE;
    c = dv < h.f64 ? -1 : (dv > h.f64 ? 1 : 0);
  } else {
    c = iv < h.i64 ? -1 : (iv > h.i64 ? 1 : 0);
  }
  switch (h.op) {
    case KHIP_OP_GT: return c > 0;
    case KHIP_OP_GE: return c >= 0;
    case KHIP_OP_LT: return c < 0;
    case KHIP_OP_LE: return c <= 0;
    case KHIP_OP_EQ: return c == 0;
    case KHIP_OP_NE: return c != 0;
  }
  return false;
}


__global__ void k_blockmax(const int64_t* __restrict__ ts, const uint8_t* __restrict__ kv,
                           const uint8_t* __restrict__ rv, int64_t n, int64_t* __restrict__ blockmax,
                           const int64_t* __restrict__ st_at);
__global__ void k_scan_blocks(const int64_t* __restrict__ blockmax, int64_t nb, int64_t* __restrict__ prefix,
                              int64_t* __restrict__ stream_time);
__global__ void k_scan_excl(int64_t* __restrict__ v, int64_t n, int64_t* __restrict__ total);
__global__ void k_compact(const uint64_t* __restrict__ table, int64_t cap, int sw, HavingDev h,
                          uint64_t* __restrict__ out, int64_t max_rows, unsigned long long* __restrict__ counter);

__global__ void k_part_colsum(const uint32_t* __restrict__ hist, int64_t nT, int P, int TC, int64_t* __restrict__ csum);
__global__ void k_part_colbase(int64_t* __restrict__ csum, int P, int TC, int64_t* __restrict__ R);
__global__ void k_part_colprefix(uint32_t* __restrict__ hist, int64_t nT, int P, int TC,
                                 const int64_t* __restrict__ csum, const int64_t* __restrict__ pbase, int pstride);

struct InitWords {
  int64_t w[32];
};

constexpr int PINFO_CTR_WORDS = 13, PINFO_CI_WORDS = 24;
struct PushInfo {
  int64_t wr[6];
  unsigned long long ctr[PINFO_CTR_WORDS];
  int64_t c1info[PINFO_CI_WORDS];
  unsigned long long closed_n;
  int64_t seed_st;
  int64_t sup_after;
  unsigned long long having_closed;
};

struct PartState {
  int64_t P = 0;
  int log2P = 0;
  int64_t cmax = 0;
  int H = 0;
  int H_eff = 0;
  int nwords = 3;
  int lds_bytes = 0;
  DevBuf pbase, ctr, counts;
  DevBuf buf[2];
  DevBuf sel, cnt, newcnt, fail;
  DevBuf hist, tilemax, tilemin, tileprefix, tpart, scan_tmp;
  DevBuf tilekr;
  DevBuf srec;
  int rw = 2, meta_word = -1;
  uint32_t vcols = 0;
  int8_t col_word[MAX_COLS] = {-1, -1, -1, -1, -1, -1, -1, -1};
  std::vector<uint8_t> psbits;
  DevBuf work;
  int64_t scat_cap = 0;
  DevBuf closed, closed_ctr;
  DevBuf closed2, pctr;
  int64_t closed_cap = 0, closed_n = 0;
  DevBuf wr, res;
  bool res_fresh = true;
  DevBuf srecA, hcoarse, scan_tmpB, RB;
  int mH = 0, m_lds = 0, rt_off = 0, m_list_off = 0, n_cu = 256;
  int flag_off = 0;
  int64_t purged_to = INT64_MIN;
  int32_t plane_off[MAX_OPS] = {};
  int8_t plane_w64[MAX_OPS] = {};
  int8_t word_op[32] = {};
  DevBuf hcnt, hnew;
  int64_t having_total = 0;
  bool hvalid = true;
  HostBuf pinfo;
  PushInfo* info() const { return pinfo.as<PushInfo>(); }
  DevBuf c1bb, c1seg, c1info, prn;
  DevBuf c1rc, c1rp, c1ro, c1scan, c1ci;
  int64_t c1_kbase = 0;
  bool c1_kb_valid = false;
  int64_t c1_wide_n = 0;
  std::vector<uint8_t> c1psbits;
  int64_t c1ps_hmax = 0, hint_groups = 1024;
  bool last_c1 = false;
  int c1_skip = 0;
  DevBuf c1vq;
  HostBuf c1vq_h;
  bool c1_wide = false;
};

struct TaggState {
  DevBuf src;
  int64_t src_cap = 0, src_occ = 0;
  int src_sw = 8;
  int key_type = -1;
  bool dense = false;
  int64_t dbase = 0;
  KeyDict dict;
  DevBuf sid, skey, skey2, sidx, sidx2, rec, tmp, tmp2, ctr, claimed, gclaimed, blk, st_koff, st_kbytes, st_kv, st_key, shash;
};

struct SessState {
  DevBuf rows, rows2;
  int64_t n = 0;
  DevBuf skey, sidx, skey2, sidx2, st_after, ukeys, ucnt, nseg, useg, s0, cap, scap, fin, fin_pre;
  DevBuf srow, sfl, trow, crow, ctomb, keep, keep_pre, ctr, tmp, tmp2, gath, blockkr;
  int64_t nchg = 0;
};

}

using namespace khip;

struct khip_agg {
  khip_agg_desc desc{};
  std::vector<int32_t> col_types;
  std::vector<khip_agg_spec> aggs;
  int device = 0;
  hipStream_t stream = nullptr;
  int64_t grace = 0;
  int windowed = 0;
  int max_fanout = 1;
  ApplyParams ap{};
  InitWords init{};
  std::vector<AggOut> outs;
  OffResolve offs{};
  std::vector<int> out_off;
  int n_hidden = 0;
  int hid_src[MAX_COLS] = {};
  bool hid_not[MAX_COLS] = {};
  DevBuf seqbuf, nseqbuf;
  int64_t seq_base = 0;
  std::vector<int> agg_k, out_flag;
  bool has_topk = false;
  struct VarWords { int w_hi = -1, w_sq = -1; };
  std::vector<VarWords> out_var;
  bool has_var = false;
  struct PairWords { int w_n = -1, w_sx = -1, w_sy = -1, w_sxx = -1, w_syy = -1, w_sxy = -1; };
  std::vector<PairWords> out_pair;
  bool has_pair = false;
  int sw = 4;
  DevBuf table;
  int64_t cap = 0;
  int64_t occ = 0;
  DevBuf blockmax, blockprefix, partials, resume, counters, stream_time;
  DevBuf st_keys, st_ts, st_kv, st_rv, st_koff, st_kbytes;
  DevBuf st_cols[MAX_COLS], st_cval[MAX_COLS];
  DevBuf kid, khash;
  int64_t resume_n = 0;
  KeyDict dict;
  int64_t host_stream_time = -1;
  bool profile = false;
  hipEvent_t ev[8] = {};
  khip_kernel_times times{};
  int engine = 0;
  khip::HavingDev having{};
  khip::PartState part;
  khip::SessState sess;
  khip::TaggState tagg;
  int64_t retention = 0;
  bool changelog = false;
// ... 79 lines not shown
```

ksql_amd/csrc/khip_agg_part.hip:

```cpp
#include <algorithm>
#include <cstring>
#include <vector>

#include <cstdlib>

#include "khip_agg_internal.hpp"
#include "khip_part.hpp"

namespace khip {

constexpr int PT_THREADS = 1024;
constexpr int R8_NT = 512;
constexpr int W_NT = 512;
constexpr int PT_ITEMS = 64;
constexpr int AG_THREADS = 1024;
constexpr uint32_t L_CLAIM = 1u;
constexpr uint32_t L_READY = 2u;
constexpr int MAX_P_LOG2 = 15;
constexpr int SPLIT_P_LOG2 = 14;
constexpr int TC_MAX = 64;


struct ColTypes {
  int32_t t[MAX_COLS];
// ... 2900 lines not shown
    kn = d > kn ? d : kn;
  }
  if ((threadIdx.x & 63) == 0) {
    smin[threadIdx.x >> 6] = mn;
    smax[threadIdx.x >> 6] = mx;
    skx[threadIdx.x >> 6] = kx;
    skn[threadIdx.x >> 6] = kn;
  }
  __syncthreads();
  if (threadIdx.x) return;
  for (int w = 0; w < 16; w++) {
    mn = smin[w] < mn ? smin[w] : mn;
    mx = smax[w] > mx ? smax[w] : mx;
    kx = skx[w] > kx ? skx[w] : kx;
    kn = skn[w] > kn ? skn[w] : kn;
  }
  wr[2] = mn;
  wr[3] = mx;
  wr[5] = mx < 0 ? 0 : mn;
  const bool span_ok = mx < 0 || mx - mn < ((int64_t)1 << 31) - 2;
  wr[6] = 0;
  wr[7] = 0;
  if (r8_allow && tilekr && mx >= 0 && span_ok) {
    const int64_t kmin = ~kn;
    const uint64_t krange = (uint64_t)kx - (uint64_t)kmin;
    const uint64_t trange = (uint64_t)(mx - mn + 1);
    const int kb = krange ? 64 - __clzll((long long)krange) : 0;
    const int tb = 64 - __clzll((long long)trange);
    if (kb + tb <= 64) {
      wr[6] = kmin;
      wr[7] = tb;
    }
  }
  ctr[CTR_ADDED] = ctr[CTR_FAILED] = ctr[CTR_NEED] = 0ULL;
  if (closed_ctr) *closed_ctr = closed_n;
  int64_t lo = INT64_MAX, hi = INT64_MIN;
  if (mx >= 0) {
    if (windowed) {
      const int64_t l = mn - size + adv;
      lo = (int64_t)fast_udiv((uint64_t)(l > 0 ? l : 0), fd);
      hi = (int64_t)fast_udiv((uint64_t)mx, fd);
    } else {
      lo = hi = 0;
    }
  }
  if (!fresh) {
    int64_t rlo = res[0];
    const int64_t rhi = res[1];
    if (windowed && close0 != INT64_MIN && rlo != INT64_MAX) {
      const int64_t c = close0 - size;
      const int64_t lb = c >= 0 ? (int64_t)fast_udiv((uint64_t)c, fd) + 1 : 0;
      rlo = rlo > lb ? rlo : lb;
    }
    lo = rlo < lo ? rlo : lo;
    hi = rhi > hi ? rhi : hi;
  }
  const bool fits = allow && log2P >= 1 && log2P < 63;
  if (lo > hi) {
    wr[0] = 0;
    wr[1] = fits;
    wr[4] = merge_allow && fits && span_ok;
    wr[8] = 0;
    res[0] = INT64_MAX;
    res[1] = INT64_MIN;
    return;
  }
  wr[0] = lo;
  wr[1] = fits && hi - lo < ((int64_t)1 << log2P) - 1;
  wr[8] = fits && log2P >= 2 && hi - lo < ((int64_t)1 << (log2P - 1)) - 1;
  wr[4] = merge_allow && wr[1] && span_ok;
  res[0] = lo;
  res[1] = hi;
}

__global__ __launch_bounds__(256) void k_part_commit(const int64_t* __restrict__ gate, int P,
                                                     const int64_t* __restrict__ pbase,
                                                     const uint32_t* __restrict__ prn,
                                                     const uint32_t* __restrict__ plist, int nlist,
                                                     uint8_t* __restrict__ sel, int64_t* __restrict__ cnt,
                                                     unsigned long long* __restrict__ newcnt,
                                                     const uint8_t* __restrict__ fail,
                                                     unsigned long long* __restrict__ out ,
                                                     unsigned long long* __restrict__ hcnt,
                                                     unsigned long long* __restrict__ hnew) {
  if (gate && gate[4] == 0) return;
  const int k = blockIdx.x * 256 + threadIdx.x;
  int64_t added = 0, failed = 0, hdelta = 0;
  if (plist ? k < nlist : k < P) {
    const uint32_t p = plist ? plist[k] : (uint32_t)k;
    if (plist || (prn ? prn[p] != 0 : pbase[p + 1] > pbase[p])) {
      if (fail[p] == 0) {
        added = (int64_t)newcnt[p] - cnt[p];
        cnt[p] = (int64_t)newcnt[p];
        sel[p] ^= 1;
        if (hcnt) {
          hdelta = (int64_t)hnew[p] - (int64_t)hcnt[p];
          hcnt[p] = hnew[p];
        }
      } else {
        failed = 1;
      }
      newcnt[p] = 0;
      if (hnew) hnew[p] = 0;
    }
  }
  added = wave_sum(added);
  failed = wave_sum(failed);
  hdelta = wave_sum(hdelta);
  if ((threadIdx.x & 63) == 0) {
    if (added) atomicAdd(&out[CTR_ADDED], (unsigned long long)added);
    if (failed) atomicAdd(&out[CTR_FAILED], (unsigned long long)failed);
    if (hdelta) atomicAdd(&out[CTR_HAVING_LIVE], (unsigned long long)hdelta);
  }
}

__global__ __launch_bounds__(256) void k_part_stats(const int64_t* __restrict__ tpart, int64_t nT,
                                                    const unsigned long long* __restrict__ closed_n,
                                                    const int64_t* __restrict__ stream_time,
                                                    unsigned long long* __restrict__ out) {
  __shared__ unsigned long long acc[T_NPART];
  if (threadIdx.x < T_NPART) acc[threadIdx.x] = 0;
  __syncthreads();
  for (int k = 0; k < T_NPART; k++) {
    int64_t v = 0;
    for (int64_t t = threadIdx.x; t < nT; t += 256) v += tpart[t * T_NPART + k];
    v = wave_sum(v);
    if ((threadIdx.x & 63) == 0 && v) atomicAdd(&acc[k], (unsigned long long)v);
  }
  __syncthreads();
  if (threadIdx.x < T_NPART) out[CTR_TILE + threadIdx.x] = acc[threadIdx.x];
  if (threadIdx.x == 0) {
    out[CTR_CLOSED] = closed_n ? *closed_n : 0ULL;
    out[CTR_STREAM_TIME] = (unsigned long long)*stream_time;
  }
}

__global__ __launch_bounds__(256) void k_part_regrow(const uint64_t* __restrict__ b0, const uint64_t* __restrict__ b1,
                                                     const uint8_t* __restrict__ sel, const int64_t* __restrict__ cnt,
                                                     int64_t ocmax, uint64_t* __restrict__ nb0, int64_t ncmax, int sw) {
  const int64_t p = blockIdx.x;
  const uint64_t* src = (sel[p] ? b1 : b0) + (uint64_t)p * ocmax * sw;
  uint64_t* dst = nb0 + (uint64_t)p * ncmax * sw;
  const int64_t words = cnt[p] * sw;
  for (int64_t w = threadIdx.x; w < words; w += 256) dst[w] = src[w];
}

__global__ __launch_bounds__(256) void k_part_regrow_flags(const uint8_t* __restrict__ f, const int64_t* __restrict__ cnt,
                                                           int64_t ocmax, uint8_t* __restrict__ nf, int64_t ncmax) {
  const int64_t p = blockIdx.x;
  for (int64_t r = threadIdx.x; r < cnt[p]; r += 256) nf[p * ncmax + r] = f[p * ocmax + r];
}

__global__ __launch_bounds__(256) void k_part_split(const uint64_t* __restrict__ b0, const uint64_t* __restrict__ b1,
                                                    const uint8_t* __restrict__ sel, const int64_t* __restrict__ cnt,
                                                    int64_t cmax, int sw, int new_log2P, uint64_t* __restrict__ nb,
                                                    int64_t ncmax, int64_t* __restrict__ ncnt) {
  __shared__ unsigned int lc[2];
  const int64_t p = blockIdx.x;
  if (threadIdx.x < 2) lc[threadIdx.x] = 0;
  __syncthreads();
  const uint64_t* src = (sel[p] ? b1 : b0) + (uint64_t)p * cmax * sw;
  for (int64_t r = threadIdx.x; r < cnt[p]; r += 256) {
    const uint64_t* row = src + r * sw;
    const uint32_t child = part_of((int64_t)row[0], new_log2P);
    const unsigned k = atomicAdd(&lc[child & 1], 1u);
    if (!nb) continue;
    uint64_t* dst = nb + ((uint64_t)child * ncmax + k) * sw;
    for (int w = 0; w < sw; w++) dst[w] = row[w];
  }
// ... 106 lines not shown
khip_status part_init(khip_agg* a, int64_t hint) {
  PartState& s = a->part;
  int used = 3;
  for (int o = 0; o < a->ap.n_ops; o++)
    used = std::max(used, op_word(a->ap.ops[o]) + op_span(a->ap, a->ap.ops[o]));
  s.nwords = used;
  const int entry = 4 + 8 * used;
  const int64_t budget = knob("KHIP_LDS_KB", 150) * 1024;
  int H = 256;
  while ((int64_t)(H * 2) * entry + 16 <= budget && H < 16384) H *= 2;
  s.H = H;
  s.H_eff = H * 3 / 4;
  s.lds_bytes = (int)((((size_t)H * 4 + 15) & ~(size_t)15) + (size_t)H * 8 * used);
  if (a->changelog) {
    s.flag_off = s.lds_bytes;
    s.lds_bytes += H;
  }
  {
    int n64 = 0, n32 = 0;
    for (int o = 0; o < a->ap.n_ops; o++) (a->ap.ops[o].kind == OP_INC || a->ap.ops[o].kind == OP_INC_VALID ? n32 : n64)++;
    const int mentry = 8 + 8 * n64 + 4 + 4 * n32 + 2;
    const int64_t mbudget = knob("KHIP_MERGE_LDS_KB", 76) * 1024;
    int mH = (int)std::min<int64_t>(16384, mbudget / mentry - 64) & ~63;
    s.mH = mH;
    const int ms = mH + 64;
    int off = ms * 8;
    for (int o = 0; o < a->ap.n_ops; o++)
      if (!(a->ap.ops[o].kind == OP_INC || a->ap.ops[o].kind == OP_INC_VALID)) {
        s.plane_off[o] = off;
        s.plane_w64[o] = 1;
        off += ms * 8;
      }
    s.rt_off = off;
    off += ms * 4;
    for (int o = 0; o < a->ap.n_ops; o++)
      if (a->ap.ops[o].kind == OP_INC || a->ap.ops[o].kind == OP_INC_VALID) {
        s.plane_off[o] = off;
        s.plane_w64[o] = 0;
        off += ms * 4;
      }
    s.m_list_off = off;
    off += (mH * 2 + 15) & ~15;
    s.m_lds = off;
    for (int w = 0; w < 32; w++) s.word_op[w] = -1;
    for (int o = 0; o < a->ap.n_ops; o++) s.word_op[op_word(a->ap.ops[o])] = (int8_t)o;
    if (mH >= 256) s.H_eff = std::min(s.H_eff, mH * 3 / 4);
  }
  const int64_t groups = std::max<int64_t>(hint, 1024);
  s.hint_groups = groups;
  s.log2P = std::min(SPLIT_P_LOG2, std::max(8, part_ceil_log2(groups * 2 / s.H_eff)));
  if (s.log2P == SPLIT_P_LOG2 && groups >> SPLIT_P_LOG2 > (int64_t)s.H_eff * 7 / 10) s.log2P = MAX_P_LOG2;
  s.log2P = (int)std::min<int64_t>(MAX_P_LOG2, knob("KHIP_PART_LOG2", s.log2P));
  s.P = 1LL << s.log2P;
  s.cmax = next_pow2(std::max<int64_t>(64, 2 * groups / s.P + 64));
  int s0 = 0;
  while (s0 < 12 && groups / s.P > ((int64_t)s.H_eff * 7 / 10) << s0) s0++;
  s.psbits.assign(s.P, (uint8_t)s0);
  bool colref[MAX_COLS] = {false};
  s.vcols = 0;
  for (int o = 0; o < a->ap.n_ops; o++) {
    if (a->ap.ops[o].kind == OP_INC) continue;
    s.vcols |= 1u << a->ap.ops[o].col;
    if (a->ap.ops[o].kind != OP_INC_VALID) colref[a->ap.ops[o].col] = true;
    if (op_is_pair(a->ap.ops[o])) {
      s.vcols |= 1u << op_col2(a->ap.ops[o]);
      colref[op_col2(a->ap.ops[o])] = true;
    }
  }
  const bool meta = a->desc.window_kind == KHIP_WINDOW_HOPPING || s.vcols != 0;
  s.meta_word = meta ? 2 : -1;
  int w = meta ? 3 : 2;
  for (int c = 0; c < MAX_COLS; c++) s.col_word[c] = (c < a->ap.n_cols && colref[c]) ? (int8_t)w++ : (int8_t)-1;
  s.rw = (w + 1) & ~1;
  KHIP_TRY(s.sel.ensure(s.P));
  KHIP_TRY(s.fail.ensure(s.P));
  KHIP_TRY(s.cnt.ensure(s.P * 8));
  KHIP_TRY(s.newcnt.ensure(s.P * 8));
  KHIP_TRY(s.pbase.ensure((s.P + 1) * 8));
  {
    int ncu = 0;
    if (hipDeviceGetAttribute(&ncu, hipDeviceAttributeMultiprocessorCount, a->device) == hipSuccess && ncu > 0)
      s.n_cu = ncu;
  }
  KHIP_TRY(s.ctr.ensure(CTR_ALLOC * 8));
  KHIP_TRY(s.hcnt.ensure(s.P * 8));
  KHIP_TRY(s.hnew.ensure(s.P * 8));
  KHIP_TRY(s.pinfo.ensure(sizeof(PushInfo)));
  KHIP_TRY_HIP(hipMemsetAsync(s.hcnt.p, 0, s.P * 8, a->stream));
  KHIP_TRY_HIP(hipMemsetAsync(s.hnew.p, 0, s.P * 8, a->stream));
  KHIP_TRY_HIP(hipMemsetAsync(s.ctr.p, 0, CTR_ALLOC * 8, a->stream));
  s.having_total = 0;
  s.hvalid = true;
  for (int b = 0; b < 2; b++) KHIP_TRY(s.buf[b].ensure((size_t)s.P * s.cmax * a->sw * 8));
  if (a->changelog) KHIP_TRY(a->chg.ensure((size_t)s.P * s.cmax));
  KHIP_TRY_HIP(hipMemsetAsync(s.sel.p, 0, s.P, a->stream));
  KHIP_TRY_HIP(hipMemsetAsync(s.fail.p, 0, s.P, a->stream));
  KHIP_TRY_HIP(hipMemsetAsync(s.cnt.p, 0, s.P * 8, a->stream));
  KHIP_TRY_HIP(hipMemsetAsync(s.newcnt.p, 0, s.P * 8, a->stream));
  return KHIP_OK;
}

void part_release(khip_agg* a) {
  PartState& s = a->part;
  s.pinfo.release();
  s.c1vq_h.release();
  DevBuf* bufs[] = {&s.hcnt, &s.hnew, &s.srecA, &s.hcoarse, &s.scan_tmpB, &s.RB, &s.wr, &s.res, &s.closed, &s.closed_ctr, &s.closed2, &s.pctr, &s.buf[0], &s.buf[1], &s.sel, &s.cnt, &s.newcnt, &s.fail, &s.hist,
                    &s.tilemax, &s.tilemin, &s.tilekr,
                    &s.tileprefix, &s.tpart, &s.scan_tmp, &s.srec, &s.work,
                    &s.c1rc, &s.c1rp, &s.c1ro, &s.c1scan, &s.c1ci, &s.c1bb, &s.c1seg, &s.c1info, &s.prn, &s.c1vq,
                    &s.pbase, &s.ctr, &s.counts};
  for (DevBuf* b : bufs) b->release();
}

__global__ __launch_bounds__(256) void k_part_reset(int64_t P, unsigned long long* __restrict__ hcnt,
                                                    unsigned long long* __restrict__ hnew, int64_t* __restrict__ cnt,
                                                    unsigned long long* __restrict__ newcnt, uint8_t* __restrict__ fail,
                                                    unsigned long long* __restrict__ ctr,
                                                    int64_t* __restrict__ stream_time) {
  const int64_t p = (int64_t)blockIdx.x * 256 + threadIdx.x;
  if (p < P) {
    hcnt[p] = 0;
    hnew[p] = 0;
    cnt[p] = 0;
    newcnt[p] = 0;
    fail[p] = 0;
  }
  if (p < CTR_ALLOC) ctr[p] = 0;
  if (p == 0) *stream_time = -1;
}

khip_status part_reset(khip_agg* a) {
  PartState& s = a->part;
  s.closed_n = 0;
  s.purged_to = INT64_MIN;
  s.res_fresh = true;
  s.hvalid = true;
  s.having_total = 0;
  s.last_c1 = false;
  s.c1_skip = 0;
  hipLaunchKernelGGL(k_part_reset, dim3(ceil_div(std::max<int64_t>(s.P, CTR_ALLOC), 256)), dim3(256), 0, a->stream, s.P,
                     s.hcnt.as<unsigned long long>(), s.hnew.as<unsigned long long>(), s.cnt.as<int64_t>(),
                     s.newcnt.as<unsigned long long>(), s.fail.as<uint8_t>(), s.ctr.as<unsigned long long>(),
                     a->stream_time.as<int64_t>());
  KHIP_TRY_HIP(hipGetLastError());
  return KHIP_OK;
}

static PartAggParams part_params(const khip_agg* a) {
  const PartState& s = a->part;
  PartAggParams q{};
  q.windowed = a->windowed;
  q.nwords = s.nwords;
  q.sw = a->sw;
  q.H = s.H;
  q.H_eff = s.H_eff;
  q.rw = s.rw;
  q.meta_word = s.meta_word;
  for (int c = 0; c < MAX_COLS; c++) q.col_word[c] = s.col_word[c];
  q.size = a->desc.size_ms;
  q.adv = a->windowed ? a->desc.advance_ms : 1;
  q.fd = make_fastdiv((uint64_t)q.adv);
  q.dbg_mode = (int32_t)knob("KHIP_AGG_MODE", 0);
  q.log2P = s.log2P;
  q.cmax = s.cmax;
  q.n_cols = a->ap.n_cols;
  q.n_ops = a->ap.n_ops;
  for (int c = 0; c < MAX_COLS; c++) q.col_type[c] = a->ap.col_type[c];
  for (int o = 0; o < a->ap.n_ops; o++) q.ops[o] = a->ap.ops[o];
  q.init = a->init;
  q.having = a->having;
  q.flag_off = a->changelog ? s.flag_off : 0;
  q.chg = a->changelog ? a->chg.as<uint8_t>() : nullptr;
  return q;
}

khip_status part_regrow(khip_agg* a, int64_t ncmax) {
  PartState& s = a->part;
  DevBuf nb[2], nchg;
  for (int b = 0; b < 2; b++) KHIP_TRY(nb[b].ensure((size_t)s.P * ncmax * a->sw * 8));
  hipLaunchKernelGGL(k_part_regrow, dim3(s.P), dim3(256), 0, a->stream, s.buf[0].as<uint64_t>(),
                     s.buf[1].as<uint64_t>(), s.sel.as<uint8_t>(), s.cnt.as<int64_t>(), s.cmax, nb[0].as<uint64_t>(),
                     ncmax, a->sw);
  KHIP_TRY_HIP(hipGetLastError());
  if (a->changelog) {
    KHIP_TRY(nchg.ensure((size_t)s.P * ncmax));
    hipLaunchKernelGGL(k_part_regrow_flags, dim3(s.P), dim3(256), 0, a->stream, a->chg.as<uint8_t>(), s.cnt.as<int64_t>(),
                       s.cmax, nchg.as<uint8_t>(), ncmax);
    KHIP_TRY_HIP(hipGetLastError());
  }
  KHIP_TRY_HIP(hipMemsetAsync(s.sel.p, 0, s.P, a->stream));
  KHIP_TRY_HIP(hipStreamSynchronize(a->stream));
  for (int b = 0; b < 2; b++) s.buf[b] = std::move(nb[b]);
// ... 46 lines not shown
  s.hvalid = false;
  KHIP_TRY(s.pbase.ensure((s.P + 1) * 8));
  return KHIP_OK;
}

static void agg_probe_report(DevBuf& b, int nb) {
  std::vector<unsigned long long> t((size_t)nb * 6 + 8);
  if (hipMemcpy(t.data(), b.p, t.size() * 8, hipMemcpyDeviceToHost) != hipSuccess) return;
  unsigned long long lo = ~0ULL, hi = 0;
  double ph[5] = {0, 0, 0, 0, 0};
  int m = 0;
  for (int i = 0; i < nb; i++) {
    const unsigned long long* r = &t[(size_t)i * 6];
    if (!r[0] || !r[5]) continue;
    m++;
    lo = std::min(lo, r[0]);
    hi = std::max(hi, r[5]);
    for (int k = 0; k < 5; k++) ph[k] += (double)(r[k + 1] - r[k]);
  }
  if (!m) return;
  fprintf(stderr, "[agg probe] %d/%d wgs, span %.1f us, avg per wg (us): phases %.2f %.2f %.2f %.2f %.2f "
          "(k_part_agg: init resident records write drain; k_part_merge: init records mark+reserve write drain)\n",
          m, nb, (hi - lo) / 100.0, ph[0] / m / 100, ph[1] / m / 100, ph[2] / m / 100, ph[3] / m / 100, ph[4] / m / 100);
}


khip_status part_grow_closed(khip_agg* a) {
  PartState& s = a->part;
  const int64_t live = a->occ - s.closed_n;
  if (s.closed_cap >= s.closed_n + live) return KHIP_OK;
  const int64_t ncap = next_pow2(std::max<int64_t>(1024, s.closed_n + live));
  DevBuf nc;
  KHIP_TRY(nc.ensure((size_t)ncap * a->sw * 8));
  if (s.closed_n)
    KHIP_TRY_HIP(hipMemcpyAsync(nc.p, s.closed.p, (size_t)s.closed_n * a->sw * 8, hipMemcpyDeviceToDevice, a->stream));
  KHIP_TRY_HIP(hipStreamSynchronize(a->stream));
  s.closed = std::move(nc);
  s.closed_cap = ncap;
  return KHIP_OK;
}

khip_status part_upload_plan(khip_agg* a, const std::vector<uint32_t>& image) {
  PartState& s = a->part;
  KHIP_TRY(s.work.ensure(image.size() * 4));
  KHIP_TRY_HIP(hipMemcpyAsync(s.work.p, image.data(), image.size() * 4, hipMemcpyHostToDevice, a->stream));
  return KHIP_OK;
}

khip_status part_plan_retry(khip_agg* a, RetryPlan& r, int pass, const std::vector<uint8_t>& host_fail) {
  PartState& s = a->part;
  if (pass > 24) return fail(KHIP_E_DEVICE, "partitioned aggregation could not place the batch");
  KHIP_TRY_HIP(hipMemsetAsync(s.fail.p, 0, s.P, a->stream));
  if (!retry_next(r, host_fail.data(), (int)s.P))
    return fail(KHIP_E_DEVICE, "partition needs more than 4096 sub-passes (extreme key skew)");
  if (r.grow) {
    const int64_t need = (int64_t)s.info()->ctr[CTR_NEED];
    KHIP_TRY(part_regrow(a, next_pow2(std::max<int64_t>(s.cmax * 2, need * 5 / 4 + 64))));
  }
  return part_upload_plan(a, r.image);
}

void part_retry_trace_counts(const RetryPlan& r, bool listed, const std::vector<uint8_t>& host_fail, int64_t* nsub,
                             int64_t* fail_table, int64_t* fail_region) {
  *nsub = *fail_table = *fail_region = 0;
  if (listed)
    for (const uint32_t x : r.work) *nsub += work_sbits(x) != 0;
  for (const uint8_t f : host_fail) *fail_table += (f & FAIL_TABLE) != 0, *fail_region += (f & FAIL_REGION) != 0;
}

void part_push_epilogue(khip_agg* a, int64_t closed_now, int64_t added, int64_t* tot) {
  PartState& s = a->part;
  const unsigned long long* c = s.info()->ctr;
  s.having_total = (int64_t)(c[CTR_HAVING_LIVE] + c[CTR_HAVING_CLOSED]);
  added += closed_now - s.closed_n;
  s.closed_n = closed_now;
  a->host_stream_time = (int64_t)c[CTR_STREAM_TIME];
  static_assert(P_ACCEPTED == T_ACCEPTED && P_NULL_KEY == T_NULL_KEY && P_NULL_ROW == T_NULL_ROW &&
                P_BAD_TS == T_BAD_TS && P_APPLIED == T_APPLIED && P_LATE == T_LATE, "tile counter k is tot[k]");
  for (int k = 0; k < T_NPART; k++) tot[k] += (int64_t)c[CTR_TILE + k];
  tot[P_NEW] += added;
}

khip_status part_pass_commit(khip_agg* a, int pass, const RetryPlan& r, const int64_t* gate, const uint32_t* prn,
                             const unsigned long long* closed_ctr, int64_t nT) {
  PartState& s = a->part;
  const int P = (int)s.P, nl = pass == 0 ? P : (int)r.plist.size();
  hipLaunchKernelGGL(k_part_commit, dim3(ceil_div(std::max(nl, 1), 256)), dim3(256), 0, a->stream, gate, P,
                     s.pbase.as<int64_t>(), prn, pass == 0 ? nullptr : s.work.as<uint32_t>() + r.work.size(), nl,
                     s.sel.as<uint8_t>(), s.cnt.as<int64_t>(), s.newcnt.as<unsigned long long>(),
                     s.fail.as<uint8_t>(), s.ctr.as<unsigned long long>(), s.hcnt.as<unsigned long long>(),
                     s.hnew.as<unsigned long long>());
  KHIP_TRY_HIP(hipGetLastError());
  if (pass == 0) {
    ev_record_part(a, 3);
    hipLaunchKernelGGL(k_part_stats, dim3(1), dim3(256), 0, a->stream, s.tpart.as<int64_t>(), nT, closed_ctr,
                       a->stream_time.as<int64_t>(), s.ctr.as<unsigned long long>());
  }
  KHIP_TRY_HIP(hipMemcpyAsync(s.info()->ctr, s.ctr.p, CTR_COPIED * 8, hipMemcpyDeviceToHost, a->stream));
  return KHIP_OK;
}

khip_status part_pass_failed(khip_agg* a, std::vector<uint8_t>* host_fail) {
  PartState& s = a->part;
  host_fail->clear();
  if (s.info()->ctr[CTR_FAILED] == 0) return KHIP_OK;
  host_fail->resize(s.P);
  KHIP_TRY_HIP(hipMemcpy(host_fail->data(), s.fail.p, s.P, hipMemcpyDeviceToHost));
  return KHIP_OK;
}


struct PartIn {
  const int64_t *keys, *ts;
  const uint8_t *kv, *rv;
  const ColPtrs* cols;
  const int64_t* st_at;
};

struct PartGeo {
  int64_t n, tile, nT, ncap;
  int P, TC, pad;
  bool lvl2, narrow;
  int fbits, B, nbins;
  int U, wu, r8u;
  bool stage, wstage, r8k, wk;
  bool rstage, rwstage;
  int ru, G, refine_mode;
  int64_t ng, ref_grid;
  bool merge_allow, r12_ok, r12_merge, cnt1, c1_plan, r8_allow;
  int mt, c1h, c1au, merge_wpc;
  int fan, pane, merge_dbg;
  size_t hist_lds, scat_lds, sw_lds, s8_lds, ref_lds, r8_lds, merge_lds;
  PartAggParams q0;
  int64_t close0;
  bool probe, trace;
};

static PartGeo part_plan(const khip_agg* a, int64_t n) {
  const PartState& s = a->part;
  PartGeo g{};
  g.n = n;
  g.P = (int)s.P;
  int64_t items = PT_ITEMS;
  while (items > 4 && ceil_div(n, (int64_t)PT_THREADS * items) < s.n_cu &&
         ceil_div(n, (int64_t)PT_THREADS * (items >> 1)) * s.P <= (1LL << 21))
    items >>= 1;
  g.tile = (int64_t)PT_THREADS * knob("KHIP_TILE_ITEMS", items);
  g.pad = (int)knob("KHIP_PAD", 0);
  g.nT = ceil_div(n, g.tile);
  g.TC = (int)std::min<int64_t>(g.nT, TC_MAX);
  g.ncap = g.pad ? n + 3 * (int64_t)g.P * g.nT : n;
  g.lvl2 = !g.pad && s.log2P >= 11 && knob("KHIP_SCATTER2", 1) != 0;
  g.fbits = g.lvl2 ? s.log2P - s.log2P / 2 : 0;
  g.B = g.P >> g.fbits;
  g.nbins = g.lvl2 ? g.B : g.P;
  g.narrow = s.rw == 2;
  g.q0 = part_params(a);
  g.close0 = (a->windowed && a->host_stream_time >= 0) ? a->host_stream_time - a->grace : INT64_MIN;
  g.merge_allow = s.mH >= 256 && knob("KHIP_MERGE", 1) != 0 && !a->has_topk && !a->has_var && !a->has_pair;
  const int64_t r12_mode = knob("KHIP_R12", 1);
  g.r12_ok = g.narrow && !g.pad && g.merge_allow && r12_mode != 0;
  g.r12_merge = g.r12_ok && (r12_mode == 1 || !g.lvl2);
  g.cnt1 = a->ap.n_ops == 1 && a->ap.ops[0].kind == OP_INC && a->ap.ops[0].word == 3 && a->sw == 4 && s.rw == 2 &&
           a->desc.window_kind != KHIP_WINDOW_HOPPING;
  g.mt = (int)knob("KHIP_MERGE_THREADS", 512);
  g.c1_plan = g.cnt1 && g.r12_merge && a->windowed && g.q0.adv <= (int64_t)1 << 31 && g.mt >= 512 &&
              knob("KHIP_MERGE_C1", 1) != 0;
  g.r8_allow = g.c1_plan && knob("KHIP_R8", 1) != 0;
  g.c1h = (int)knob("KHIP_C1_LOG2H", 12);
  g.c1au = (int)knob("KHIP_C1_AU", 6);
  g.merge_wpc = (int)knob("KHIP_MERGE_WG_PER_CU", g.c1_plan ? 2 : (g.mt >= 512 ? KHIP_MG_WPE / 2 : KHIP_MG_WPE));
  g.merge_lds = g.c1_plan ? (size_t)((1 << g.c1h) + 64) * 16 : (size_t)s.m_lds;
  g.fan = a->windowed ? (int32_t)std::min<int64_t>((g.q0.size + g.q0.adv - 1) / g.q0.adv, 1 << 20) : 1;
  g.pane = a->windowed && g.fan > 1 && g.fan <= MG_FB && g.q0.size % g.q0.adv == 0 && knob("KHIP_PANES", 1) ? 1 : 0;
  g.merge_dbg = (int)knob("KHIP_MERGE_DEBUG", 0);
  const int U = (int)knob("KHIP_SCATTER_U", g.narrow ? 8 : 16);
  g.U = U >= 16 ? 16 : (U >= 8 ? 8 : (g.narrow && U >= 6 ? 6 : 4));
  const bool stage_knob = knob("KHIP_STAGE", 1) != 0, wstage_knob = knob("KHIP_WSTAGE", 1) != 0;
  g.stage = g.narrow && !g.pad && g.nbins <= PT_THREADS && g.U <= 8 && stage_knob;
  g.wstage = !g.narrow && s.rw == 4 && !g.pad && g.nbins <= PT_THREADS && wstage_knob;
  g.wu = g.U >= 16 ? 4 : 2;
// ... 225 lines not shown
  cq.log2H = g.c1h;
  cq.sw = mq.sw;
  cq.size = mq.size;
  cq.adv = mq.adv;
  cq.fd = mq.fd;
  cq.fd32 = mq.fd32;
  cq.hv_active = a->having.active;
  cq.hv_op = a->having.op;
  cq.hv_i64 = a->having.i64;
  return cq;
}

static void part_launch_agg(khip_agg* a, const PartGeo& g, const PartAggQ& k, bool merge, int pass, const uint32_t* wk,
                            int64_t nwork, unsigned long long* dbg) {
  PartState& s = a->part;
  unsigned long long* ctr = s.ctr.as<unsigned long long>();
  const int first = pass == 0 ? 1 : 0, lds = (int)g.merge_lds;
  const int64_t grid = std::min<int64_t>(nwork, (int64_t)s.n_cu * g.merge_wpc);
  if (merge && g.c1_plan) {
    const int au = g.c1au;
    for (int rm = g.r8_allow ? 1 : 0; rm >= 0; rm--) {
      auto mk = rm ? (au >= 8 ? k_part_merge_c1<512, 8, 1> : (au >= 6 ? k_part_merge_c1<512, 6, 1> : k_part_merge_c1<512, 4, 1>))
                   : (au >= 8 ? k_part_merge_c1<512, 8, 0> : (au >= 6 ? k_part_merge_c1<512, 6, 0> : k_part_merge_c1<512, 4, 0>));
      hipFuncSetAttribute((const void*)mk, hipFuncAttributeMaxDynamicSharedMemorySize, lds);
      hipLaunchKernelGGL(mk, dim3(grid), dim3(512), lds, a->stream, k.cq, wk, nwork, s.pbase.as<int64_t>(),
                         s.srec.as<uint64_t>(), first, s.buf[0].as<uint64_t>(), s.buf[1].as<uint64_t>(),
                         s.sel.as<uint8_t>(), s.cnt.as<int64_t>(), s.newcnt.as<unsigned long long>(),
                         s.fail.as<uint8_t>(), ctr + CTR_NEED, g.close0, s.closed.as<uint64_t>(),
                         s.closed_ctr.as<unsigned long long>(), s.wr.as<int64_t>(), s.hnew.as<unsigned long long>(),
                         ctr + CTR_HAVING_CLOSED, dbg);
    }
  } else if (merge) {
    const bool cnt1 = g.cnt1;
    auto mk = k.mq.r12 ? (g.mt >= 512 ? (cnt1 ? k_part_merge<true, 512, true> : k_part_merge<false, 512, true>)
                                       : (cnt1 ? k_part_merge<true, 256, true> : k_part_merge<false, 256, true>))
                       : (g.mt >= 512 ? (cnt1 ? k_part_merge<true, 512, false> : k_part_merge<false, 512, false>)
                                       : (cnt1 ? k_part_merge<true, 256, false> : k_part_merge<false, 256, false>));
    hipFuncSetAttribute((const void*)mk, hipFuncAttributeMaxDynamicSharedMemorySize, lds);
    hipLaunchKernelGGL(mk, dim3(grid), dim3(g.mt >= 512 ? 512 : 256), lds, a->stream, k.mq, wk, nwork,
                       s.pbase.as<int64_t>(), s.srec.as<uint64_t>(), first, s.buf[0].as<uint64_t>(),
                       s.buf[1].as<uint64_t>(), s.sel.as<uint8_t>(), s.cnt.as<int64_t>(),
                       s.newcnt.as<unsigned long long>(), s.fail.as<uint8_t>(), ctr + CTR_NEED, g.close0,
                       s.closed.as<uint64_t>(), s.closed_ctr.as<unsigned long long>(), s.wr.as<int64_t>(),
                       s.hnew.as<unsigned long long>(), ctr + CTR_HAVING_CLOSED, dbg);
  } else {
    hipFuncSetAttribute((const void*)k_part_agg, hipFuncAttributeMaxDynamicSharedMemorySize, s.lds_bytes);
    hipLaunchKernelGGL(k_part_agg, dim3(nwork), dim3(AG_THREADS), s.lds_bytes, a->stream, k.q, wk, s.pbase.as<int64_t>(),
                       s.srec.as<uint64_t>(), first, s.buf[0].as<uint64_t>(), s.buf[1].as<uint64_t>(),
                       s.sel.as<uint8_t>(), s.cnt.as<int64_t>(), s.newcnt.as<unsigned long long>(),
                       s.fail.as<uint8_t>(), ctr + CTR_NEED, g.close0, s.closed.as<uint64_t>(),
                       s.closed_ctr.as<unsigned long long>(), s.wr.as<int64_t>(), dbg);
  }
}

static void merge_probe_report(const khip_agg* a, const PartGeo& g, const DevBuf& b) {
  unsigned long long ph[8] = {};
  if (hipMemcpy(ph, b.p, sizeof(ph), hipMemcpyDeviceToHost) != hipSuccess) return;
  const double us = (double)std::min<int64_t>(g.P, 2 * a->part.n_cu) * 100.0;
  if (g.c1_plan)
    fprintf(stderr, "[merge c1 probe] per workgroup (us): item start+evict %.1f records %.1f mark+count+reserve %.1f "
            "write %.1f\n", ph[0] / us, ph[1] / us, ph[2] / us, ph[3] / us);
  else
    fprintf(stderr, "[merge probe] per workgroup (us): setup %.1f evict %.1f records %.1f mark+reserve %.1f write %.1f\n",
            ph[0] / us, ph[1] / us, ph[2] / us, ph[3] / us, ph[4] / us);
}

static khip_status part_run_pass(khip_agg* a, const PartGeo& g, PartAggQ& k, const RetryPlan& r, bool subs0, bool merge,
                                 int pass, DevBuf& dbgbuf, int64_t* nwork, unsigned long long** dbg) {
  PartState& s = a->part;
  const uint32_t* wk = (pass == 0 && !subs0) ? nullptr : s.work.as<uint32_t>();
  *nwork = wk ? (int64_t)r.work.size() : g.P;
  *dbg = nullptr;
  if (g.probe && pass == 0) {
    KHIP_TRY(dbgbuf.ensure((size_t)std::max<int64_t>(g.P, (int64_t)r.work.size()) * 6 * 8 + 64));
    KHIP_TRY_HIP(hipMemsetAsync(dbgbuf.p, 0, dbgbuf.bytes, a->stream));
    *dbg = dbgbuf.as<unsigned long long>();
  }
  k.q.cmax = k.mq.cmax = k.cq.cmax = s.cmax;
  k.q.chg = k.mq.chg = k.cq.chg = a->changelog ? a->chg.as<uint8_t>() : nullptr;
  if (pass > 0) KHIP_TRY_HIP(hipMemsetAsync(s.ctr.p, 0, CTR_PER_PASS * 8, a->stream));
  part_launch_agg(a, g, k, merge, pass, wk, *nwork, *dbg);
  KHIP_TRY(part_pass_commit(a, pass, r, (merge && pass == 0) ? s.wr.as<int64_t>() : (const int64_t*)nullptr, nullptr,
                            a->windowed ? s.closed_ctr.as<unsigned long long>() : (const unsigned long long*)nullptr,
                            g.nT));
  KHIP_TRY_HIP(hipStreamSynchronize(a->stream));
  return KHIP_OK;
}

#ifdef KHIP_TUNING
static void part_trace_plan(const khip_agg* a, const PartGeo& g) {
  fprintf(stderr,
          "[part plan] rw=%d P=%d tile=%lld nT=%lld lvl2=%d fbits=%d stage=%d wstage=%d r8k=%d wk=%d r12=%d cnt1=%d "
          "c1_plan=%d r8_allow=%d merge_allow=%d U=%d\n",
          a->part.rw, g.P, (long long)g.tile, (long long)g.nT, g.lvl2 ? 1 : 0, g.fbits, g.stage ? 1 : 0,
          g.wstage ? 1 : 0, g.r8k ? 1 : 0, g.wk ? 1 : 0, g.r12_ok ? (g.r12_merge ? 1 : 2) : 0, g.cnt1 ? 1 : 0,
          g.c1_plan ? 1 : 0, g.r8_allow ? 1 : 0, g.merge_allow ? 1 : 0, g.U);
}

static void part_trace_pass(const khip_agg* a, const PartGeo& g, const RetryPlan& r, bool merge, int pass, bool listed,
                            int64_t nwork, const std::vector<uint8_t>& host_fail) {
  const PartState& s = a->part;
  const unsigned long long* c2 = s.info()->ctr;
  int64_t nsub, ft, fr;
  part_retry_trace_counts(r, listed, host_fail, &nsub, &ft, &fr);
  const int H = !merge ? s.H : (g.c1_plan ? 1 << g.c1h : s.mH);
  fprintf(stderr,
          "[part trace] kernel=%s P=%d cmax=%lld H=%d pass=%d items=%lld sub_items=%lld failed=%llu "
          "fail_table=%lld fail_region=%lld closed_before=%lld closed_after=%llu\n",
          !merge ? "agg" : (g.c1_plan ? "merge_c1" : "merge"), g.P, (long long)s.cmax, H, pass, (long long)nwork,
          (long long)nsub, c2[CTR_FAILED], (long long)ft, (long long)fr, (long long)s.closed_n,
          a->windowed ? c2[CTR_CLOSED] : 0ULL);
}
#endif

static khip_status part_split_crowded(khip_agg* a) {
  PartState& s = a->part;
  while (s.log2P < SPLIT_P_LOG2 && a->occ - s.closed_n > s.P * (int64_t)s.H_eff / 2) KHIP_TRY(part_split(a));
  return KHIP_OK;
}

static khip_status part_try_pipeline(khip_agg* a, int64_t n, const C1In& in, int64_t* tot, bool* done) {
  bool declined = false;
  KHIP_TRY(c1_push(a, n, in, tot, &declined));
  if (a->profile) (declined ? a->times.c1_declined : a->times.c1_pushes)++;
  if (declined) a->part.c1_skip = 8;
  *done = !declined;
  return KHIP_OK;
}

khip_status part_push_rows(khip_agg* a, int64_t n, const RowsIn& ri, int key_col, int64_t* tot, bool* done,
                           bool supplied) {
  PartState& s = a->part;
  *done = false;
  KHIP_TRY(part_split_crowded(a));
  s.last_c1 = false;
  int vcol = -1;
  if (s.c1_skip > 0 || !c1v_eligible(a, n, &vcol)) return KHIP_OK;
  RowsIn r = ri;
  r.vword = vcol == key_col ? 0 : 2 + vcol - (vcol > key_col ? 1 : 0);
  r.vbit = vcol;
  const int64_t* st_flag = supplied ? (const int64_t*)ri.rows : nullptr;
  return part_try_pipeline(a, n, C1In{nullptr, nullptr, nullptr, nullptr, st_flag, nullptr, vcol, &r}, tot, done);
}

khip_status part_push(khip_agg* a, int64_t n, const int64_t* keys, const int64_t* ts, const uint8_t* kv,
                      const uint8_t* rv, const ColPtrs& cols, int64_t* tot, const int64_t* st_at) {
  PartState& s = a->part;
  KHIP_TRY(part_split_crowded(a));
  s.last_c1 = false;
  int vcol = -1;
  if (s.c1_skip > 0) {
    s.c1_skip--;
  } else if (c1_eligible(a, n) || c1v_eligible(a, n, &vcol)) {
    bool done = false;
    KHIP_TRY(part_try_pipeline(a, n, C1In{keys, ts, kv, rv, st_at, vcol >= 0 ? &cols : nullptr, vcol, nullptr}, tot,
                               &done));
    if (done) return KHIP_OK;
  }
  const PartIn in{keys, ts, kv, rv, &cols, st_at};
  const PartGeo g = part_plan(a, n);
#ifdef KHIP_TUNING
  if (g.trace) part_trace_plan(a, g);
#endif
  KHIP_TRY(part_scratch(a, g));
  KHIP_TRY(part_histogram(a, in, g));
  part_offsets(a, g);
  KHIP_TRY(part_scatter(a, in, g));
// ... 196 lines not shown
```

ksql_amd/csrc/khip_part.hpp:

```cpp
#pragma once

#include "khip_agg_internal.hpp"
#include "khip_retry.hpp"

namespace khip {

enum { T_ACCEPTED, T_NULL_KEY, T_NULL_ROW, T_BAD_TS, T_APPLIED, T_LATE, T_NPART };

enum {
  CTR_ADDED = 0,
  CTR_FAILED = 1,
  CTR_NEED = 2,
  CTR_TILE = 3,
  CTR_PER_PASS = CTR_TILE,
  CTR_CLOSED = CTR_TILE + T_NPART,
  CTR_STREAM_TIME,
  CTR_HAVING_LIVE,
  CTR_HAVING_CLOSED,
  CTR_COPIED,
  CTR_ALLOC = 16
};
static_assert(CTR_HAVING_LIVE == 11 && CTR_HAVING_CLOSED == 12, "the counter block's layout");
static_assert(CTR_COPIED == PINFO_CTR_WORDS && CTR_COPIED <= CTR_ALLOC, "the counter copy fits its buffers");
constexpr unsigned long long C1_FATAL = 1ULL << 63;

enum {
  CI_KMIN = 0,
  CI_KMAX = 1,
  CI_TFAIL = 2,
  CI_T0 = 3,
  CI_GATE = 4,
  CI_WBASE = 5,
  CI_WBITS = 6,
  CI_ID32 = 7,
  CI_TMIN = 8,
  CI_TMAX = 9,
  CI_KBITS = 10,
  CI_NCHUNK = 11,
  CI_KMINC = 12,
  CI_WHI = 13,
  CI_KRANGE = 14,
  CI_WIDE = 15,
  CI_REASON = 16,
  CI_FITS = 17,
  CI_KBASE = 18,
  CI_KSHIFT = 19,
  CI_KFAIL = 20,
  CI_N = 24
};
static_assert(CI_N == PINFO_CI_WORDS, "PushInfo holds a c1info copy");

__device__ __forceinline__ uint64_t key_hash(int64_t key) { return mix64((uint64_t)key ^ 0x6A09E667F3BCC908ULL); }

__device__ __forceinline__ int64_t key_of_hash(uint64_t h) {
  h ^= h >> 33;
  h *= 0x9cb4b2f8129337dbULL;
  h ^= h >> 33;
  h *= 0x4f74430c22a54005ULL;
  h ^= h >> 33;
  return (int64_t)(h ^ 0x6A09E667F3BCC908ULL);
}

constexpr uint64_t EMPTY_ID = ~0ULL;

__device__ __forceinline__ uint32_t part_of_hk(uint64_t hk, int log2P) {
  return log2P == 0 ? 0u : (uint32_t)(hk >> (64 - log2P));
}

__device__ __forceinline__ uint32_t part_of(int64_t key, int log2P) { return part_of_hk(key_hash(key), log2P); }

__device__ __forceinline__ int64_t tile_of(int64_t b, int64_t nT) {
  const int64_t per = nT / 8, rem = nT % 8, x = b % 8, k = b / 8;
  return x * per + (x < rem ? x : rem) + k;
}

__device__ __forceinline__ void lds_barrier() {
  asm volatile("s_waitcnt lgkmcnt(0)\n\ts_barrier" ::: "memory");
}

#define KLDS __attribute__((address_space(3)))
typedef KLDS uint32_t lds_u32;
typedef KLDS int64_t lds_i64;
typedef KLDS double lds_f64;
#define WG_RLX __ATOMIC_RELAXED, __HIP_MEMORY_SCOPE_WORKGROUP

constexpr uint32_t RT_MATCHED = 0x80000000u;

__device__ __forceinline__ void mg_list_append(bool claimed, uint32_t e, KLDS uint16_t* nl, int* nnew) {
  const uint64_t b = __ballot(claimed);
  if (!b) return;
  const int lane = threadIdx.x & 63, leader = __ffsll((long long)b) - 1;
  int base = 0;
  if (lane == leader) base = atomicAdd(nnew, __popcll(b));
  base = __shfl(base, leader, 64);
  if (claimed) nl[base + __popcll(b & ((1ULL << lane) - 1))] = (uint16_t)e;
}

template <int AU>
__device__ __forceinline__ int mg_list_append_n(const bool (&claimed)[AU], const uint32_t (&e)[AU], KLDS uint16_t* nl,
                                                int* nnew) {
  uint64_t b[AU];
  int tot = 0;
#pragma unroll
  for (int u = 0; u < AU; u++) {
    b[u] = __ballot(claimed[u]);
    tot += __popcll(b[u]);
  }
  if (!tot) return 0;
  const int lane = threadIdx.x & 63;
  int base = 0;
  if (lane == 0) base = atomicAdd(nnew, tot);
  base = __builtin_amdgcn_readfirstlane(base);
  const uint64_t lt = (1ULL << lane) - 1;
#pragma unroll
  for (int u = 0; u < AU; u++) {
    if (claimed[u]) nl[base + __popcll(b[u] & lt)] = (uint16_t)e[u];
    base += __popcll(b[u]);
  }
  return base;
}

constexpr uint32_t C1_GOLD = 0x9E3779B1u;

__device__ __forceinline__ uint32_t stage_bin(uint64_t hk, int shift, uint32_t mask) {
  return shift >= 64 ? 0u : (uint32_t)(hk >> shift) & mask;
}

struct StageR8 {
  uint32_t* cur;
  uint32_t* cnt;
  uint32_t* sbase;
  uint32_t* gpos;
  int64_t* sp;
  uint16_t* sbin;
  int* wsum;
};

__host__ __device__ constexpr size_t stage_r8_lds_bytes(int nb, int S) {
  return (size_t)nb * 16 + (size_t)S * 8 + ((size_t)S * 2 + 15) / 16 * 16;
}

__device__ __forceinline__ StageR8 stage_r8_carve(char* smem, int nb, int S, int* wsum) {
  StageR8 L;
  L.cur = (uint32_t*)smem;
  L.cnt = L.cur + nb;
  L.sbase = L.cnt + nb;
  L.gpos = L.sbase + nb;
  L.sp = (int64_t*)(smem + (size_t)nb * 16);
  L.sbin = (uint16_t*)(L.sp + S);
  L.wsum = wsum;
  return L;
}

template <int U, int NT>
__device__ __forceinline__ void stage_step_r8(const int64_t (&rec)[U], const uint32_t (&bin)[U], const bool (&ok)[U],
                                              int nb, const StageR8& L, uint64_t* __restrict__ srec) {
  const int t = threadIdx.x, lane = t & 63, wave = t >> 6;
  uint32_t rank[U];
#pragma unroll
  for (int u = 0; u < U; u++) rank[u] = ok[u] ? atomicAdd(&L.cnt[bin[u]], 1u) : 0u;
  lds_barrier();
  const uint32_t c = t < nb ? L.cnt[t] : 0u;
  uint32_t incl = c;
  for (int off = 1; off < 64; off <<= 1) {
    const uint32_t y = __shfl_up(incl, off, 64);
    if (lane >= off) incl += y;
  }
  if (lane == 63) L.wsum[wave] = (int)incl;
  lds_barrier();
  uint32_t before = 0, tot = 0;
#pragma unroll
  for (int k = 0; k < NT / 64; k++) {
    before += k < wave ? (uint32_t)L.wsum[k] : 0u;
    tot += (uint32_t)L.wsum[k];
  }
  if (t < nb) {
    L.sbase[t] = before + incl - c;
    L.gpos[t] = L.cur[t];
    L.cur[t] += c;
    L.cnt[t] = 0u;
  }
  lds_barrier();
#pragma unroll
  for (int u = 0; u < U; u++)
    if (ok[u]) {
      const uint32_t i = L.sbase[bin[u]] + rank[u];
      L.sp[i] = rec[u];
      L.sbin[i] = (uint16_t)bin[u];
    }
  lds_barrier();
  for (uint32_t j = t; j < tot; j += NT) {
    const uint32_t b = L.sbin[j];
    srec[(uint64_t)L.gpos[b] + (j - L.sbase[b])] = (uint64_t)L.sp[j];
  }
}

__global__ void k_part_pscan(int64_t* __restrict__ v, int64_t n);
__global__ void k_part_stats(const int64_t* __restrict__ tpart, int64_t nT, const unsigned long long* __restrict__ closed_n,
                             const int64_t* __restrict__ stream_time, unsigned long long* __restrict__ out);
khip_status part_grow_closed(khip_agg* a);
khip_status part_upload_plan(khip_agg* a, const std::vector<uint32_t>& image);
khip_status part_plan_retry(khip_agg* a, RetryPlan& r, int pass, const std::vector<uint8_t>& host_fail);
void part_retry_trace_counts(const RetryPlan& r, bool listed, const std::vector<uint8_t>& host_fail, int64_t* nsub,
                             int64_t* fail_table, int64_t* fail_region);
khip_status part_pass_commit(khip_agg* a, int pass, const RetryPlan& r, const int64_t* gate, const uint32_t* prn,
                             const unsigned long long* closed_ctr, int64_t nT);
khip_status part_pass_failed(khip_agg* a, std::vector<uint8_t>* host_fail);
void part_push_epilogue(khip_agg* a, int64_t closed_now, int64_t added, int64_t* tot);
bool c1_eligible(khip_agg* a, int64_t n);
bool c1v_eligible(khip_agg* a, int64_t n, int* col);
struct C1In {
  const int64_t *keys, *ts;
  const uint8_t *kv, *rv;
  const int64_t* st_at;
  const ColPtrs* cols;
  int vcol;
  const RowsIn* rows;
};
khip_status c1_push(khip_agg* a, int64_t n, const C1In& in, int64_t* tot, bool* declined);
__global__ void k_part_commit(const int64_t* __restrict__ gate, int P, const int64_t* __restrict__ pbase,
                              const uint32_t* __restrict__ prn, const uint32_t* __restrict__ plist, int nlist,
                              uint8_t* __restrict__ sel, int64_t* __restrict__ cnt,
                              unsigned long long* __restrict__ newcnt, const uint8_t* __restrict__ fail,
                              unsigned long long* __restrict__ out, unsigned long long* __restrict__ hcnt,
                              unsigned long long* __restrict__ hnew);

}
```

Baseline: 55.99 billion.

## Store per-tile u16 run offsets plus tile totals instead of u32 run positions

```diff
diff --git a/ksql_amd/csrc/khip_agg_c1.hip b/ksql_amd/csrc/khip_agg_c1.hip
--- a/ksql_amd/csrc/khip_agg_c1.hip
+++ b/ksql_amd/csrc/khip_agg_c1.hip
@@ -4,7 +4,6 @@
 #include <vector>
 
 #include "khip_part.hpp"
-#include "khip_sort.hpp"
 
 namespace khip {
 
@@ -105,30 +104,39 @@
 
 template <int SPT, int NT>
 __device__ __forceinline__ void flush_run_counts(const uint32_t* lrc, const uint16_t* lro, int B, int st_last, int64_t t,
-                                                 int64_t nSt, uint32_t* __restrict__ rcnt, uint16_t* __restrict__ roff) {
+                                                 int64_t nT, uint16_t* __restrict__ rloc, uint16_t* __restrict__ roff,
+                                                 uint32_t* __restrict__ ttot) {
   static_assert(SPT % 8 == 0, "whole 16-byte stores");
+  static_assert(C1_TILE - C1_TILE / SPT < 65536, "a run's place within its tile fits a u16");
+  const int64_t nSt = nT * SPT;
   for (int b = threadIdx.x; b < B; b += NT) {
-    uint32_t* rc = rcnt + (int64_t)b * nSt + t * SPT;
+    uint16_t* rl = rloc + (int64_t)b * nSt + t * SPT;
     uint16_t* ro = roff + (int64_t)b * nSt + t * SPT;
-#pragma unroll
-    for (int q = 0; q < SPT / 4; q++) {
-      uint32_t v[4];
-#pragma unroll
-      for (int k = 0; k < 4; k++) v[k] = 4 * q + k <= st_last ? lrc[(4 * q + k) * B + b] : 0u;
-      *(uint4*)(rc + 4 * q) = make_uint4(v[0], v[1], v[2], v[3]);
-    }
+    uint32_t acc = 0u;
 #pragma unroll
     for (int q = 0; q < SPT / 8; q++) {
-      uint32_t w[4];
+      uint32_t v[4], w[4];
 #pragma unroll
       for (int k = 0; k < 4; k++) {
         const int s0 = 8 * q + 2 * k;
+        const uint32_t p0 = acc;
+        acc += s0 <= st_last ? lrc[s0 * B + b] : 0u;
+        const uint32_t p1 = acc;
+        acc += s0 + 1 <= st_last ? lrc[(s0 + 1) * B + b] : 0u;
+        v[k] = p0 | p1 << 16;
         const uint32_t lo = s0 <= st_last ? lro[s0 * B + b] : 0u, hi = s0 + 1 <= st_last ? lro[(s0 + 1) * B + b] : 0u;
         w[k] = lo | hi << 16;
       }
+      *(uint4*)(rl + 8 * q) = make_uint4(v[0], v[1], v[2], v[3]);
       *(uint4*)(ro + 8 * q) = make_uint4(w[0], w[1], w[2], w[3]);
     }
-  }
+    ttot[(int64_t)b * nT + t] = acc;
+  }
+}
+
+__device__ __forceinline__ int64_t run_pos(const uint32_t* __restrict__ tb, const uint16_t* __restrict__ rl, int64_t nSt,
+                                           int sh, int64_t s) {
+  return (int64_t)tb[s >> sh] + (s < nSt ? (int64_t)rl[s] : 0);
 }
 
 __device__ __forceinline__ void run_bases(const int64_t* __restrict__ keys, const int64_t* __restrict__ ts, int64_t n,
@@ -155,8 +163,8 @@
 template <int U, int NT, bool WIDE, bool ST>
 __global__ __launch_bounds__(NT) __attribute__((amdgpu_waves_per_eu(4))) void k_c1_scatter(
     const int64_t* __restrict__ keys, const int64_t* __restrict__ ts, const uint8_t* __restrict__ kv,
-    const uint8_t* __restrict__ rv, int64_t n, int64_t nT, int log2B, uint32_t* __restrict__ rcnt,
-    uint16_t* __restrict__ roff, int64_t nSt, uint64_t* __restrict__ srec, int64_t* __restrict__ tilestat,
+    const uint8_t* __restrict__ rv, int64_t n, int64_t nT, int log2B, uint16_t* __restrict__ rloc,
+    uint16_t* __restrict__ roff, uint32_t* __restrict__ ttot, uint64_t* __restrict__ srec, int64_t* __restrict__ tilestat,
     int64_t* __restrict__ tpart, int64_t* __restrict__ ci, const int64_t* __restrict__ st_at,
     uint32_t* __restrict__ srecT, int64_t size, int64_t adv, FastDiv fd, int64_t grace,
     const int64_t* __restrict__ stream_time, int64_t kb_in, int has_kb) {
@@ -281,7 +289,7 @@
     }
     if (threadIdx.x == 0 && st > 0) publish(s0 - S, st - 1);
   }
-  flush_run_counts<SPT, NT>(lrc, lro, B, st_last, t, nSt, rcnt, roff);
+  flush_run_counts<SPT, NT>(lrc, lro, B, st_last, t, nT, rloc, roff, ttot);
   if (!WIDE && kor) lkfail = 1;
   __syncthreads();
   if (threadIdx.x == 0 && s0 > base) publish(s0 - S, st_last);
@@ -333,14 +341,40 @@
   }
 }
 
-__global__ __launch_bounds__(256) void k_c1_bases(const uint32_t* __restrict__ rpos, int64_t nSt, int B,
-                                                  int64_t* __restrict__ bb) {
-  for (int b = threadIdx.x; b <= B; b += blockDim.x) bb[b] = (int64_t)rpos[(int64_t)b * nSt];
-}
-
-__global__ __launch_bounds__(256) void k_c1_chunks(const int* __restrict__ cstart, int B, const int64_t* __restrict__ bb,
-                                                   const uint32_t* __restrict__ rpos, int64_t nSt, int ch,
-                                                   const int64_t* __restrict__ ci, uint32_t* __restrict__ cinfo) {
+__global__ __launch_bounds__(1024) void k_c1_runpos(const uint32_t* __restrict__ ttot, int64_t nT,
+                                                    uint32_t* __restrict__ tbase) {
+  __shared__ uint32_t wsum[16];
+  const int lane = threadIdx.x & 63, wave = threadIdx.x >> 6;
+  const uint32_t* in = ttot + (int64_t)blockIdx.x * nT;
+  uint32_t* out = tbase + (int64_t)blockIdx.x * (nT + 1);
+  uint32_t carry = 0u;
+  for (int64_t t0 = 0; t0 < nT; t0 += 1024) {
+    const int64_t t = t0 + threadIdx.x;
+    const uint32_t c = t < nT ? in[t] : 0u;
+    uint32_t incl = c;
+    for (int off = 1; off < 64; off <<= 1) {
+      const uint32_t y = __shfl_up(incl, off, 64);
+      if (lane >= off) incl += y;
+    }
+    if (lane == 63) wsum[wave] = incl;
+    __syncthreads();
+    uint32_t before = 0u, tot = 0u;
+#pragma unroll
+    for (int k = 0; k < 16; k++) {
+      before += k < wave ? wsum[k] : 0u;
+      tot += wsum[k];
+    }
+    if (t < nT) out[t] = carry + before + incl - c;
+    carry += tot;
+    __syncthreads();
+  }
+  if (threadIdx.x == 0) out[nT] = carry;
+}
+
+__global__ __launch_bounds__(256) void k_c1_chunks(const int* __restrict__ cstart, int B,
+                                                   const uint32_t* __restrict__ tbase, const uint16_t* __restrict__ rloc,
+                                                   int64_t nT, int sh, int ch, const int64_t* __restrict__ ci,
+                                                   uint32_t* __restrict__ cinfo) {
   if (ci_ld(ci, CI_GATE) == 0) return;
   const int w = blockIdx.x * blockDim.x + threadIdx.x;
   if (w >= (int)ci_ld(ci, CI_NCHUNK)) return;
@@ -351,32 +385,43 @@
     else e = m;
   }
   const int b = a;
-  const int64_t lo = bb[b] + (int64_t)(w - cstart[b]) * ch;
-  const int64_t len = bb[b + 1] - lo < ch ? bb[b + 1] - lo : ch;
-  const uint32_t* rp = rpos + (int64_t)b * nSt;
-  int64_t sa = 0, se = nSt;
-  while (se - sa > 1) {
-    const int64_t m = (sa + se) >> 1;
-    if ((int64_t)rp[m] <= lo) sa = m;
-    else se = m;
-  }
-  int64_t ta = sa, te = nSt;
-  while (te - ta > 1) {
-    const int64_t m = (ta + te) >> 1;
-    if ((int64_t)rp[m] < lo + len) ta = m;
-    else te = m;
+  const int64_t nSt = nT << sh, spt = (int64_t)1 << sh;
+  const uint32_t* tb = tbase + (int64_t)b * (nT + 1);
+  const uint16_t* rl = rloc + (int64_t)b * nSt;
+  const int64_t lo = (int64_t)(w - cstart[b]) * ch, blen = (int64_t)tb[nT];
+  const int64_t hi = blen - lo < ch ? blen : lo + ch;
+  int64_t t0 = 0, e0 = nT, t1 = 0, e1 = nT;
+  while (e0 - t0 > 1 || e1 - t1 > 1) {
+    const int64_t m0 = (t0 + e0) >> 1, m1 = (t1 + e1) >> 1;
+    const int64_t p0 = (int64_t)tb[m0], p1 = (int64_t)tb[m1];
+    if (e0 - t0 > 1) {
+      if (p0 <= lo) t0 = m0;
+      else e0 = m0;
+    }
+    if (e1 - t1 > 1) {
+      if (p1 < hi) t1 = m1;
+      else e1 = m1;
+    }
+  }
+  const int64_t b0 = (int64_t)tb[t0], b1 = (int64_t)tb[t1];
+  int64_t sa = t0 << sh, sl = t1 << sh;
+  for (int64_t half = spt >> 1; half > 0; half >>= 1) {
+    const int64_t q0 = b0 + (int64_t)rl[sa + half], q1 = b1 + (int64_t)rl[sl + half];
+    if (q0 <= lo) sa += half;
+    if (q1 < hi) sl += half;
   }
   cinfo[2 * w] = (uint32_t)sa;
-  cinfo[2 * w + 1] = (uint32_t)(te - sa);
-}
-
-__device__ __forceinline__ void chunk_map(const uint32_t* __restrict__ rp, const uint16_t* __restrict__ ro,
+  cinfo[2 * w + 1] = (uint32_t)(sl + 1 - sa);
+}
+
+__device__ __forceinline__ void chunk_map(const uint32_t* __restrict__ tb, const uint16_t* __restrict__ rl,
+                                          const uint16_t* __restrict__ ro, int64_t nSt, int sh,
                                           const uint32_t* __restrict__ cinfo, int w, int64_t S, int64_t lo, int len,
                                           uint32_t* map) {
   const int64_t s0 = cinfo[2 * w];
   const int R = (int)cinfo[2 * w + 1];
   for (int k = threadIdx.x; k < R; k += blockDim.x) {
-    const int64_t s = s0 + k, p = (int64_t)rp[s], pe = (int64_t)rp[s + 1];
+    const int64_t s = s0 + k, p = run_pos(tb, rl, nSt, sh, s), pe = run_pos(tb, rl, nSt, sh, s + 1);
     const int64_t a = p > lo ? p : lo, e = pe < lo + len ? pe : lo + len;
     const uint32_t src = (uint32_t)(s * S + (int64_t)ro[s] + (a - p));
     for (int64_t x = a; x < e; x++) map[x - lo] = src + (uint32_t)(x - a);
@@ -385,17 +430,22 @@
 }
 
 __global__ __launch_bounds__(1024) void k_c1_check(
-    const int64_t* __restrict__ tilestat, int64_t nT, int64_t size, int64_t adv, FastDiv fd, int64_t grace,
-    int64_t close0, int fresh, int log2B, int log2P, int wide, int ch, int kbmax, int pbits,
-    const int64_t* __restrict__ bb, int* __restrict__ cstart,
+    const int64_t* __restrict__ tilestat, const int64_t* __restrict__ tpart, int64_t nT, int64_t size, int64_t adv,
+    FastDiv fd, int64_t grace, int64_t close0, int fresh, int log2B, int log2P, int wide, int ch, int kbmax, int pbits,
+    const uint32_t* __restrict__ tbase, int64_t* __restrict__ bb, int* __restrict__ cstart,
     int64_t* __restrict__ ci, int64_t* __restrict__ stream_time, int64_t* __restrict__ res,
     unsigned long long* __restrict__ ctr, unsigned long long* __restrict__ closed_ctr, unsigned long long closed_n) {
   __shared__ int64_t wmx[16];
-  __shared__ int64_t red[4][16];
+  __shared__ int64_t red[2][16];
+  __shared__ unsigned long long lsum[T_NPART];
   __shared__ int lslow;
-  __shared__ int lnch[512 + 1];
+  __shared__ int64_t wtot[8];
+  __shared__ int wnch[8], wmxc[8];
   const int lane = threadIdx.x & 63, wave = threadIdx.x >> 6;
   if (threadIdx.x == 0) lslow = 0;
+  if (threadIdx.x < T_NPART) lsum[threadIdx.x] = 0ULL;
+  const int B = 1 << log2B;
+  const uint32_t btot = (int)threadIdx.x < B ? tbase[(int64_t)threadIdx.x * (nT + 1) + nT] : 0u;
   const int64_t st0 = *stream_time;
   const int64_t K = (nT + 1023) / 1024;
   const int64_t g0 = threadIdx.x * K, g1 = g0 + K < nT ? g0 + K : nT;
@@ -409,6 +459,7 @@
   const int64_t excl = __shfl_up(incl, 1, 64);
   int64_t run = lane == 0 ? pre : (excl > pre ? excl : pre);
   int64_t gmn = INT64_MAX, gmx = -1;
+  int64_t tsum[T_NPART] = {};
   bool slow = false;
   for (int64_t g = g0; g < g1; g++) {
     const int64_t* t4 = tilestat + 4 * g;
@@ -419,6 +470,8 @@
     }
     run = mx > run ? mx : run;
     gmx = mx > gmx ? mx : gmx;
+#pragma unroll
+    for (int k = 0; k < T_NPART; k++) tsum[k] += tpart[g * T_NPART + k];
   }
   if (slow) lslow = 1;
   for (int off = 32; off > 0; off >>= 1) {
@@ -426,24 +479,56 @@
     gmn = a < gmn ? a : gmn;
     gmx = b > gmx ? b : gmx;
   }
+#pragma unroll
+  for (int k = 0; k < T_NPART; k++) tsum[k] = wave_sum(tsum[k]);
   if (lane == 0) {
     red[0][wave] = gmn;
     red[1][wave] = gmx;
-  }
-  const int B = 1 << log2B;
-  for (int b = threadIdx.x; b < B; b += 1024) lnch[b] = (int)((bb[b + 1] - bb[b] + ch - 1) / ch);
+#pragma unroll
+    for (int k = 0; k < T_NPART; k++)
+      if (tsum[k]) atomicAdd(&lsum[k], (unsigned long long)tsum[k]);
+  }
+  const int nch = (int)((btot + (uint32_t)ch - 1u) / (uint32_t)ch);
+  int64_t itot = (int64_t)btot;
+  int inch = nch, mnch = nch;
+  for (int off = 1; off < 64; off <<= 1) {
+    const int64_t y = __shfl_up(itot, off, 64);
+    const int z = __shfl_up(inch, off, 64), q = __shfl_xor(mnch, off, 64);
+    if (lane >= off) {
+      itot += y;
+      inch += z;
+    }
+    mnch = q > mnch ? q : mnch;
+  }
+  if (lane == 63 && wave < 8) {
+    wtot[wave] = itot;
+    wnch[wave] = inch;
+    wmxc[wave] = mnch;
+  }
   __syncthreads();
+  if ((int)threadIdx.x < B) {
+    int64_t bt = 0;
+    int bn = 0;
+    for (int w = 0; w < wave; w++) {
+      bt += wtot[w];
+      bn += wnch[w];
+    }
+    bb[threadIdx.x] = bt + itot - (int64_t)btot;
+    cstart[threadIdx.x] = bn + inch - nch;
+  }
   if (threadIdx.x) return;
   for (int w = 0; w < 16; w++) {
     gmn = red[0][w] < gmn ? red[0][w] : gmn;
     gmx = red[1][w] > gmx ? red[1][w] : gmx;
   }
   int acc = 0, mxc = 0;
-  for (int b = 0; b < B; b++) {
-    cstart[b] = acc;
-    acc += lnch[b];
-    mxc = lnch[b] > mxc ? lnch[b] : mxc;
-  }
+  int64_t base = 0;
+  for (int w = 0; w < 8; w++) {
+    base += wtot[w];
+    acc += wnch[w];
+    mxc = wmxc[w] > mxc ? wmxc[w] : mxc;
+  }
+  bb[B] = base;
   cstart[B] = acc;
   const int64_t kmin = ci_ld(ci, CI_KMIN), kmax = ci_ld(ci, CI_KMAX);
   const bool tfail = ci_ld(ci, CI_TFAIL) != 0, kfail = ci_ld(ci, CI_KFAIL) != 0;
@@ -502,6 +587,7 @@
   res[0] = none ? INT64_MAX : lo;
   res[1] = none ? INT64_MIN : hi;
   ctr[CTR_ADDED] = ctr[CTR_FAILED] = ctr[CTR_NEED] = 0ULL;
+  for (int k = 0; k < T_NPART; k++) ctr[CTR_TILE + k] = lsum[k];
   if (closed_ctr) *closed_ctr = closed_n;
 }
 
@@ -509,8 +595,9 @@
 __global__ __launch_bounds__(NT) __attribute__((amdgpu_waves_per_eu(4))) void k_c1_refine(
     const uint64_t* __restrict__ srcA, const int64_t* __restrict__ bb, const int* __restrict__ cstart, int log2B,
     int log2P, int fbits, uint64_t* __restrict__ srec, uint16_t* __restrict__ seg, const int64_t* __restrict__ ci,
-    const uint32_t* __restrict__ srcAT, uint32_t* __restrict__ srecT, const uint32_t* __restrict__ rpos,
-    const uint16_t* __restrict__ roff, int64_t nSt, int64_t S, const uint32_t* __restrict__ cinfo) {
+    const uint32_t* __restrict__ srcAT, uint32_t* __restrict__ srecT, const uint32_t* __restrict__ tbase,
+    const uint16_t* __restrict__ rloc, const uint16_t* __restrict__ roff, int64_t nT, int sh, int64_t S,
+    const uint32_t* __restrict__ cinfo) {
   if (ci_ld(ci, CI_GATE) == 0) return;
   const int w = blockIdx.x;
   if (w >= (int)ci_ld(ci, CI_NCHUNK)) return;
@@ -536,9 +623,9 @@
   const int64_t kmin = ci_ld(ci, CI_KMINC);
   const uint64_t kshift = WIDE ? 0 : (uint64_t)ci_ld(ci, CI_KSHIFT) << 32;
   const int shift = 64 - log2P;
-  const uint32_t* rp = rpos + (int64_t)b * nSt;
-  const uint16_t* ro = roff + (int64_t)b * nSt;
-  chunk_map(rp, ro, cinfo, w, S, lo, len, (uint32_t*)stage);
+  const int64_t nSt = nT << sh;
+  chunk_map(tbase + (int64_t)b * (nT + 1), rloc + (int64_t)b * nSt, roff + (int64_t)b * nSt, nSt, sh, cinfo, w, S,
+            lo - bb[b], len, (uint32_t*)stage);
   uint64_t r[U];
   uint32_t f[U], rank[U], t32[U];
 #pragma unroll
@@ -1301,8 +1388,8 @@
 template <int U, int NT, bool ST, bool ROWS>
 __global__ __launch_bounds__(NT) __attribute__((amdgpu_waves_per_eu(4))) void k_c1v_scatter(
     const int64_t* __restrict__ keys, const int64_t* __restrict__ ts, const uint8_t* __restrict__ kv,
-    const uint8_t* __restrict__ rv, C1VCol vc, RowsIn ri, int64_t n, int64_t nT, int log2B, uint32_t* __restrict__ rcnt,
-    uint16_t* __restrict__ roff, int64_t nSt, ulonglong2* __restrict__ srec, int64_t* __restrict__ tilestat,
+    const uint8_t* __restrict__ rv, C1VCol vc, RowsIn ri, int64_t n, int64_t nT, int log2B, uint16_t* __restrict__ rloc,
+    uint16_t* __restrict__ roff, uint32_t* __restrict__ ttot, ulonglong2* __restrict__ srec, int64_t* __restrict__ tilestat,
     int64_t* __restrict__ tpart, int64_t* __restrict__ ci, const int64_t* __restrict__ st_at, int64_t size, int64_t adv,
     FastDiv fd, int hop, int64_t grace, const int64_t* __restrict__ stream_time, int64_t kb_in, int has_kb) {
   extern __shared__ __attribute__((aligned(16))) char smem[];
@@ -1451,7 +1538,7 @@
     }
     if (threadIdx.x == 0 && st > 0) publish(s0 - S, st - 1);
   }
-  flush_run_counts<SPT, NT>(lrc, lro, B, st_last, t, nSt, rcnt, roff);
+  flush_run_counts<SPT, NT>(lrc, lro, B, st_last, t, nT, rloc, roff, ttot);
   if (kor) lkfail = 1;
   __syncthreads();
   if (threadIdx.x == 0 && s0 > base) publish(s0 - S, st_last);
@@ -1490,8 +1577,8 @@
 __global__ __launch_bounds__(NT) __attribute__((amdgpu_waves_per_eu(4))) void k_c1v_refine(
     const ulonglong2* __restrict__ srcA, const int64_t* __restrict__ bb, const int* __restrict__ cstart, int log2B,
     int log2P, int fbits, ulonglong2* __restrict__ srec, uint16_t* __restrict__ seg, const int64_t* __restrict__ ci,
-    const uint32_t* __restrict__ rpos, const uint16_t* __restrict__ roff, int64_t nSt, int64_t S,
-    const uint32_t* __restrict__ cinfo) {
+    const uint32_t* __restrict__ tbase, const uint16_t* __restrict__ rloc, const uint16_t* __restrict__ roff,
+    int64_t nT, int sh, int64_t S, const uint32_t* __restrict__ cinfo) {
   if (ci_ld(ci, CI_GATE) == 0) return;
   const int w = blockIdx.x;
   if (w >= (int)ci_ld(ci, CI_NCHUNK)) return;
@@ -1518,9 +1605,9 @@
   const int64_t kmin = ci_ld(ci, CI_KMINC);
   const uint64_t kshift = (uint64_t)ci_ld(ci, CI_KSHIFT) << 32;
   const int shift = 64 - log2P;
-  const uint32_t* rp = rpos + (int64_t)b * nSt;
-  const uint16_t* ro = roff + (int64_t)b * nSt;
-  chunk_map(rp, ro, cinfo, w, S, lo, len, (uint32_t*)stage);
+  const int64_t nSt = nT << sh;
+  chunk_map(tbase + (int64_t)b * (nT + 1), rloc + (int64_t)b * nSt, roff + (int64_t)b * nSt, nSt, sh, cinfo, w, S,
+            lo - bb[b], len, (uint32_t*)stage);
   ulonglong2 r[U];
   uint32_t f[U], rank[U];
 #pragma unroll
@@ -2394,8 +2481,9 @@
   int* cstart;
   uint16_t* seg;
   uint32_t *srecAT, *srecT;
-  uint32_t *rc, *rp;
-  uint16_t* ro;
+  int sh;
+  uint32_t *tt, *tb;
+  uint16_t *rl, *ro;
   int64_t adv, close0;
   FastDiv fd;
 };
@@ -2426,8 +2514,11 @@
   g->nSt = g->nT * (C1_TILE / g->S);
   g->nchunk_max = ceil_div(n, g->CH) + g->B;
   const int64_t B = g->B, nSt = g->nSt, nT = g->nT;
-  KHIP_TRY(s.c1rc.ensure((size_t)B * nSt * 4));
-  KHIP_TRY(s.c1rp.ensure(((size_t)B * nSt + 1) * 4));
+  static_assert(C1_TILE / (C1V_UV * C1_NT) == 32 && C1_TILE / (8 * C1_NT) == 16, "steps per tile");
+  g->sh = g->val ? 5 : 4;
+  KHIP_TRY(s.c1rc.ensure((size_t)B * nT * 4));
+  KHIP_TRY(s.c1rp.ensure((size_t)B * (nT + 1) * 4));
+  KHIP_TRY(s.c1rl.ensure((size_t)B * nSt * 2));
   KHIP_TRY(s.c1ro.ensure((size_t)B * nSt * 2));
   KHIP_TRY(s.c1bb.ensure((size_t)(B + 1) * 8));
   g->seg_bytes = ((size_t)g->nchunk_max * (g->F + 1) * 2 + 255) & ~(size_t)255;
@@ -2443,14 +2534,7 @@
   }
   KHIP_TRY(s.srec.ensure((size_t)(n + 1) * 16));
   KHIP_TRY(s.srecA.ensure((size_t)(n + 1) * std::max(s.rw, 2) * 8));
-  if (!s.c1info.p) {
-    KHIP_TRY(s.c1info.ensure(CI_N * 8));
-    int64_t init[CI_N] = {};
-    init[CI_KMIN] = INT64_MAX;
-    init[CI_KMAX] = INT64_MIN;
-    KHIP_TRY_HIP(hipMemcpy(s.c1info.p, init, sizeof(init), hipMemcpyHostToDevice));
-  }
-  g->ci = s.c1info.as<int64_t>();
+  g->ci = s.ctr.as<int64_t>() + CTR_ALLOC;
 #ifdef KHIP_TUNING
   {
     const int64_t dbg = knob("KHIP_C1_DEBUG", 0);
@@ -2466,8 +2550,9 @@
   g->wide = !g->val && s.c1_wide;
   g->srecAT = (uint32_t*)(s.srecA.as<uint64_t>() + n + 1);
   g->srecT = (uint32_t*)(s.srec.as<uint64_t>() + n + 1);
-  g->rc = s.c1rc.as<uint32_t>();
-  g->rp = s.c1rp.as<uint32_t>();
+  g->tt = s.c1rc.as<uint32_t>();
+  g->tb = s.c1rp.as<uint32_t>();
+  g->rl = s.c1rl.as<uint16_t>();
   g->ro = s.c1ro.as<uint16_t>();
   return KHIP_OK;
 }
@@ -2488,7 +2573,7 @@
     const size_t lds = run_stage_lds(g.B, UV * C1_NT, 16, false) + run_cnt_lds(g.B, C1_TILE / (UV * C1_NT));
     if (lds > 64 * 1024) hipFuncSetAttribute((const void*)sk, hipFuncAttributeMaxDynamicSharedMemorySize, (int)lds);
     hipLaunchKernelGGL(sk, dim3(g.nT), dim3(C1_NT), lds, a->stream, in.keys, in.ts, in.kv, in.rv, vc, ri, g.n, g.nT,
-                       g.log2B, g.rc, g.ro, g.nSt, (ulonglong2*)s.srecA.p, s.tilemax.as<int64_t>(),
+                       g.log2B, g.rl, g.ro, g.tt, (ulonglong2*)s.srecA.p, s.tilemax.as<int64_t>(),
                        s.tpart.as<int64_t>(), g.ci, st_at, a->desc.size_ms, g.adv, g.fd,
                        a->desc.size_ms != g.adv ? 1 : 0, a->grace, (const int64_t*)a->stream_time.as<int64_t>(),
                        s.c1_kbase, has_kb);
@@ -2499,14 +2584,13 @@
     const size_t lds = run_stage_lds(g.B, U * C1_NT, 8, g.wide) + run_cnt_lds(g.B, C1_TILE / (U * C1_NT));
     if (lds > 64 * 1024) hipFuncSetAttribute((const void*)sk, hipFuncAttributeMaxDynamicSharedMemorySize, (int)lds);
     hipLaunchKernelGGL(sk, dim3(g.nT), dim3(C1_NT), lds, a->stream, in.keys, in.ts, in.kv, in.rv, g.n, g.nT, g.log2B,
-                       g.rc, g.ro, g.nSt, s.srecA.as<uint64_t>(), s.tilemax.as<int64_t>(), s.tpart.as<int64_t>(), g.ci,
+                       g.rl, g.ro, g.tt, s.srecA.as<uint64_t>(), s.tilemax.as<int64_t>(), s.tpart.as<int64_t>(), g.ci,
                        st_at, g.srecAT, a->desc.size_ms, g.adv, g.fd, a->grace,
                        (const int64_t*)a->stream_time.as<int64_t>(), s.c1_kbase, has_kb);
   }
   KHIP_TRY_HIP(hipGetLastError());
-  KHIP_TRY((ksort::scan_excl<uint32_t, uint32_t>(a->stream, s.c1scan, g.rc, g.rp, (int64_t)g.B * g.nSt, true, nullptr)));
-  hipLaunchKernelGGL(k_c1_bases, dim3(1), dim3(256), 0, a->stream, (const uint32_t*)g.rp, g.nSt, g.B,
-                     s.c1bb.as<int64_t>());
+  hipLaunchKernelGGL(k_c1_runpos, dim3(g.B), dim3(1024), 0, a->stream, (const uint32_t*)g.tt, g.nT, g.tb);
+  KHIP_TRY_HIP(hipGetLastError());
   ev_record_part(a, 1);
   return KHIP_OK;
 }
@@ -2519,7 +2603,7 @@
     hipFuncSetAttribute((const void*)rk, hipFuncAttributeMaxDynamicSharedMemorySize, (int)lds);
     hipLaunchKernelGGL(rk, dim3((unsigned)g.nchunk_max), dim3(C1_NT), lds, a->stream, (const ulonglong2*)s.srecA.p,
                        s.c1bb.as<int64_t>(), g.cstart, g.log2B, s.log2P, g.fbits, (ulonglong2*)s.srec.p, g.seg, g.ci,
-                       (const uint32_t*)g.rp, (const uint16_t*)g.ro, g.nSt, g.S,
+                       (const uint32_t*)g.tb, (const uint16_t*)g.rl, (const uint16_t*)g.ro, g.nT, g.sh, g.S,
                        (const uint32_t*)s.c1ci.as<uint32_t>());
   } else {
     constexpr int U = C1_CH / C1_NT;
@@ -2528,8 +2612,8 @@
     if (lds > 64 * 1024) hipFuncSetAttribute((const void*)rk, hipFuncAttributeMaxDynamicSharedMemorySize, (int)lds);
     hipLaunchKernelGGL(rk, dim3((unsigned)g.nchunk_max), dim3(C1_NT), lds, a->stream, s.srecA.as<uint64_t>(),
                        s.c1bb.as<int64_t>(), g.cstart, g.log2B, s.log2P, g.fbits, s.srec.as<uint64_t>(), g.seg, g.ci,
-                       (const uint32_t*)g.srecAT, g.srecT, (const uint32_t*)g.rp, (const uint16_t*)g.ro, g.nSt, g.S,
-                       (const uint32_t*)s.c1ci.as<uint32_t>());
+                       (const uint32_t*)g.srecAT, g.srecT, (const uint32_t*)g.tb, (const uint16_t*)g.rl,
+                       (const uint16_t*)g.ro, g.nT, g.sh, g.S, (const uint32_t*)s.c1ci.as<uint32_t>());
   }
   KHIP_TRY_HIP(hipGetLastError());
   return KHIP_OK;
@@ -2538,14 +2622,15 @@
 static khip_status c1_records(khip_agg* a, const C1In& in, const C1Geo& g) {
   PartState& s = a->part;
   KHIP_TRY(c1_scatter(a, in, g));
-  hipLaunchKernelGGL(k_c1_check, dim3(1), dim3(1024), 0, a->stream, s.tilemax.as<int64_t>(), g.nT, a->desc.size_ms,
-                     g.adv, g.fd, a->grace, g.close0, s.res_fresh ? 1 : 0, g.log2B, s.log2P, g.wide ? 1 : 0, g.CH,
-                     g.val ? 31 : 32, g.panes ? 1 : 0, s.c1bb.as<int64_t>(), g.cstart, g.ci,
-                     a->stream_time.as<int64_t>(), s.res.as<int64_t>(), s.ctr.as<unsigned long long>(),
-                     s.closed_ctr.as<unsigned long long>(), (unsigned long long)s.closed_n);
+  hipLaunchKernelGGL(k_c1_check, dim3(1), dim3(1024), 0, a->stream, s.tilemax.as<int64_t>(),
+                     (const int64_t*)s.tpart.as<int64_t>(), g.nT, a->desc.size_ms, g.adv, g.fd, a->grace, g.close0,
+                     s.res_fresh ? 1 : 0, g.log2B, s.log2P, g.wide ? 1 : 0, g.CH, g.val ? 31 : 32, g.panes ? 1 : 0,
+                     (const uint32_t*)g.tb, s.c1bb.as<int64_t>(), g.cstart, g.ci, a->stream_time.as<int64_t>(),
+                     s.res.as<int64_t>(), s.ctr.as<unsigned long long>(), s.closed_ctr.as<unsigned long long>(),
+                     (unsigned long long)s.closed_n);
   KHIP_TRY(s.c1ci.ensure((size_t)g.nchunk_max * 8));
   hipLaunchKernelGGL(k_c1_chunks, dim3((unsigned)ceil_div(g.nchunk_max, 256)), dim3(256), 0, a->stream,
-                     (const int*)g.cstart, g.B, (const int64_t*)s.c1bb.as<int64_t>(), (const uint32_t*)g.rp, g.nSt, g.CH,
+                     (const int*)g.cstart, g.B, (const uint32_t*)g.tb, (const uint16_t*)g.rl, g.nT, g.sh, g.CH,
                      (const int64_t*)g.ci, s.c1ci.as<uint32_t>());
   KHIP_TRY(c1_refine(a, g));
   ev_record_part(a, 2);
@@ -2664,12 +2749,12 @@
   bool go_wide = !g.val && hci[CI_REASON] == 1;
   if (hci[CI_REASON] == 2 && !kretried) {
     long long kr[2] = {INT64_MIN, INT64_MIN};
-    KHIP_TRY(s.c1scan.ensure(16));
-    KHIP_TRY_HIP(hipMemcpyAsync(s.c1scan.p, kr, 16, hipMemcpyHostToDevice, a->stream));
+    KHIP_TRY(s.c1kr.ensure(16));
+    KHIP_TRY_HIP(hipMemcpyAsync(s.c1kr.p, kr, 16, hipMemcpyHostToDevice, a->stream));
     hipLaunchKernelGGL(k_c1_krange, dim3((unsigned)std::min<int64_t>(ceil_div(g.n, 256), 2048)), dim3(256), 0,
                        a->stream, in.rows ? (const int64_t*)in.rows->rows : in.keys,
-                       in.rows ? (int64_t)in.rows->rw : 1, g.n, s.c1scan.as<long long>());
-    KHIP_TRY_HIP(hipMemcpyAsync(kr, s.c1scan.p, 16, hipMemcpyDeviceToHost, a->stream));
+                       in.rows ? (int64_t)in.rows->rw : 1, g.n, s.c1kr.as<long long>());
+    KHIP_TRY_HIP(hipMemcpyAsync(kr, s.c1kr.p, 16, hipMemcpyDeviceToHost, a->stream));
     KHIP_TRY_HIP(hipStreamSynchronize(a->stream));
     const int64_t kmin = (int64_t)~(uint64_t)kr[0], kmax = (int64_t)kr[1];
     if ((uint64_t)kmax - (uint64_t)kmin < (1ULL << (g.val ? 31 : 32)) - 1) {
@@ -2730,9 +2815,7 @@
       const int64_t nwork = wk ? (int64_t)r.work.size() : g.P;
       KHIP_TRY(c1_launch_merge(a, g, m, pass, wk, nwork, dbg));
       KHIP_TRY(part_pass_commit(a, pass, r, pass == 0 ? (const int64_t*)g.ci : (const int64_t*)nullptr,
-                                s.prn.as<uint32_t>(), s.closed_ctr.as<unsigned long long>(), g.nT));
-      if (pass == 0) KHIP_TRY_HIP(hipMemcpyAsync(pi->c1info, g.ci, CI_N * 8, hipMemcpyDeviceToHost, a->stream));
-      KHIP_TRY_HIP(hipMemcpyAsync(&pi->closed_n, s.closed_ctr.p, 8, hipMemcpyDeviceToHost, a->stream));
+                                s.prn.as<uint32_t>(), s.closed_ctr.as<unsigned long long>(), g.nT, true));
       KHIP_TRY_HIP(hipStreamSynchronize(a->stream));
       if (pass == 0 && pi->c1info[CI_GATE] == 0) {
         KHIP_TRY(c1_declined_next(a, in, g, kretried, &next));
@@ -2765,7 +2848,7 @@
                 "[c1 trace] val=%d P=%d cmax=%lld log2H=%d pass=%d items=%lld sub_items=%lld failed=%llu fail_table=%lld "
                 "fail_region=%lld closed_before=%lld closed_after=%llu\n",
                 g.val ? 1 : 0, g.P, (long long)s.cmax, g.val ? m.v_log2H : m.log2H, pass, (long long)nwork,
-                (long long)nsub, c2[CTR_FAILED], (long long)ft, (long long)fr, (long long)s.closed_n, pi->closed_n);
+                (long long)nsub, c2[CTR_FAILED], (long long)ft, (long long)fr, (long long)s.closed_n, c2[CTR_CLOSED]);
       }
 #endif
       if (c2[CTR_FAILED] == 0) break;
@@ -2787,7 +2870,7 @@
     retry_learn(s.c1psbits, r);
     s.res_fresh = false;
     s.last_c1 = true;
-    part_push_epilogue(a, (int64_t)pi->closed_n, added_total, tot);
+    part_push_epilogue(a, (int64_t)c2[CTR_CLOSED], added_total, tot);
     return KHIP_OK;
   }
 }
diff --git a/ksql_amd/csrc/khip_agg_internal.hpp b/ksql_amd/csrc/khip_agg_internal.hpp
--- a/ksql_amd/csrc/khip_agg_internal.hpp
+++ b/ksql_amd/csrc/khip_agg_internal.hpp
@@ -539,12 +539,11 @@
   int64_t w[32];
 };
 
-constexpr int PINFO_CTR_WORDS = 13, PINFO_CI_WORDS = 24;
+constexpr int PINFO_CTR_WORDS = 16, PINFO_CI_WORDS = 24;
 struct PushInfo {
   int64_t wr[6];
   unsigned long long ctr[PINFO_CTR_WORDS];
   int64_t c1info[PINFO_CI_WORDS];
-  unsigned long long closed_n;
   int64_t seed_st;
   int64_t sup_after;
   unsigned long long having_closed;
@@ -587,8 +586,9 @@
   bool hvalid = true;
   HostBuf pinfo;
   PushInfo* info() const { return pinfo.as<PushInfo>(); }
-  DevBuf c1bb, c1seg, c1info, prn;
-  DevBuf c1rc, c1rp, c1ro, c1scan, c1ci;
+  DevBuf c1bb, c1seg, prn;
+  DevBuf c1rc, c1rp, c1rl, c1ro, c1ci;
+  DevBuf c1kr;
   int64_t c1_kbase = 0;
   bool c1_kb_valid = false;
   int64_t c1_wide_n = 0;
diff --git a/ksql_amd/csrc/khip_agg_part.hip b/ksql_amd/csrc/khip_agg_part.hip
--- a/ksql_amd/csrc/khip_agg_part.hip
+++ b/ksql_amd/csrc/khip_agg_part.hip
@@ -3006,9 +3006,15 @@
                                                      const uint8_t* __restrict__ fail,
                                                      unsigned long long* __restrict__ out ,
                                                      unsigned long long* __restrict__ hcnt,
-                                                     unsigned long long* __restrict__ hnew) {
+                                                     unsigned long long* __restrict__ hnew,
+                                                     const unsigned long long* __restrict__ closed_n,
+                                                     const int64_t* __restrict__ stream_time) {
   if (gate && gate[4] == 0) return;
   const int k = blockIdx.x * 256 + threadIdx.x;
+  if (k == 0 && stream_time) {
+    out[CTR_CLOSED] = closed_n ? *closed_n : 0ULL;
+    out[CTR_STREAM_TIME] = (unsigned long long)*stream_time;
+  }
   int64_t added = 0, failed = 0, hdelta = 0;
   if (plist ? k < nlist : k < P) {
     const uint32_t p = plist ? plist[k] : (uint32_t)k;
@@ -3281,7 +3287,13 @@
     if (hipDeviceGetAttribute(&ncu, hipDeviceAttributeMultiprocessorCount, a->device) == hipSuccess && ncu > 0)
       s.n_cu = ncu;
   }
-  KHIP_TRY(s.ctr.ensure(CTR_ALLOC * 8));
+  KHIP_TRY(s.ctr.ensure((CTR_ALLOC + CI_N) * 8));
+  {
+    int64_t init[CI_N] = {};
+    init[CI_KMIN] = INT64_MAX;
+    init[CI_KMAX] = INT64_MIN;
+    KHIP_TRY_HIP(hipMemcpy(s.ctr.as<int64_t>() + CTR_ALLOC, init, sizeof(init), hipMemcpyHostToDevice));
+  }
   KHIP_TRY(s.hcnt.ensure(s.P * 8));
   KHIP_TRY(s.hnew.ensure(s.P * 8));
   KHIP_TRY(s.pinfo.ensure(sizeof(PushInfo)));
@@ -3306,7 +3318,7 @@
   DevBuf* bufs[] = {&s.hcnt, &s.hnew, &s.srecA, &s.hcoarse, &s.scan_tmpB, &s.RB, &s.wr, &s.res, &s.closed, &s.closed_ctr, &s.closed2, &s.pctr, &s.buf[0], &s.buf[1], &s.sel, &s.cnt, &s.newcnt, &s.fail, &s.hist,
                     &s.tilemax, &s.tilemin, &s.tilekr,
                     &s.tileprefix, &s.tpart, &s.scan_tmp, &s.srec, &s.work,
-                    &s.c1rc, &s.c1rp, &s.c1ro, &s.c1scan, &s.c1ci, &s.c1bb, &s.c1seg, &s.c1info, &s.prn, &s.c1vq,
+                    &s.c1rc, &s.c1rp, &s.c1rl, &s.c1ro, &s.c1kr, &s.c1ci, &s.c1bb, &s.c1seg, &s.prn, &s.c1vq,
                     &s.pbase, &s.ctr, &s.counts};
   for (DevBuf* b : bufs) b->release();
 }
@@ -3519,21 +3531,24 @@
 }
 
 khip_status part_pass_commit(khip_agg* a, int pass, const RetryPlan& r, const int64_t* gate, const uint32_t* prn,
-                             const unsigned long long* closed_ctr, int64_t nT) {
+                             const unsigned long long* closed_ctr, int64_t nT, bool pipeline) {
   PartState& s = a->part;
   const int P = (int)s.P, nl = pass == 0 ? P : (int)r.plist.size();
   hipLaunchKernelGGL(k_part_commit, dim3(ceil_div(std::max(nl, 1), 256)), dim3(256), 0, a->stream, gate, P,
                      s.pbase.as<int64_t>(), prn, pass == 0 ? nullptr : s.work.as<uint32_t>() + r.work.size(), nl,
                      s.sel.as<uint8_t>(), s.cnt.as<int64_t>(), s.newcnt.as<unsigned long long>(),
                      s.fail.as<uint8_t>(), s.ctr.as<unsigned long long>(), s.hcnt.as<unsigned long long>(),
-                     s.hnew.as<unsigned long long>());
+                     s.hnew.as<unsigned long long>(), closed_ctr,
+                     pipeline ? (const int64_t*)a->stream_time.as<int64_t>() : (const int64_t*)nullptr);
   KHIP_TRY_HIP(hipGetLastError());
   if (pass == 0) {
     ev_record_part(a, 3);
-    hipLaunchKernelGGL(k_part_stats, dim3(1), dim3(256), 0, a->stream, s.tpart.as<int64_t>(), nT, closed_ctr,
-                       a->stream_time.as<int64_t>(), s.ctr.as<unsigned long long>());
-  }
-  KHIP_TRY_HIP(hipMemcpyAsync(s.info()->ctr, s.ctr.p, CTR_COPIED * 8, hipMemcpyDeviceToHost, a->stream));
+    if (!pipeline)
+      hipLaunchKernelGGL(k_part_stats, dim3(1), dim3(256), 0, a->stream, s.tpart.as<int64_t>(), nT, closed_ctr,
+                         a->stream_time.as<int64_t>(), s.ctr.as<unsigned long long>());
+  }
+  const size_t words = pipeline && pass == 0 ? CTR_ALLOC + CI_N : CTR_COPIED;
+  KHIP_TRY_HIP(hipMemcpyAsync(s.info()->ctr, s.ctr.p, words * 8, hipMemcpyDeviceToHost, a->stream));
   return KHIP_OK;
 }
 
@@ -3925,7 +3940,7 @@
   part_launch_agg(a, g, k, merge, pass, wk, *nwork, *dbg);
   KHIP_TRY(part_pass_commit(a, pass, r, (merge && pass == 0) ? s.wr.as<int64_t>() : (const int64_t*)nullptr, nullptr,
                             a->windowed ? s.closed_ctr.as<unsigned long long>() : (const unsigned long long*)nullptr,
-                            g.nT));
+                            g.nT, false));
   KHIP_TRY_HIP(hipStreamSynchronize(a->stream));
   return KHIP_OK;
 }
diff --git a/ksql_amd/csrc/khip_part.hpp b/ksql_amd/csrc/khip_part.hpp
--- a/ksql_amd/csrc/khip_part.hpp
+++ b/ksql_amd/csrc/khip_part.hpp
@@ -21,7 +21,7 @@
   CTR_ALLOC = 16
 };
 static_assert(CTR_HAVING_LIVE == 11 && CTR_HAVING_CLOSED == 12, "the counter block's layout");
-static_assert(CTR_COPIED == PINFO_CTR_WORDS && CTR_COPIED <= CTR_ALLOC, "the counter copy fits its buffers");
+static_assert(CTR_ALLOC == PINFO_CTR_WORDS && CTR_COPIED <= CTR_ALLOC, "the counter copy fits its buffers");
 constexpr unsigned long long C1_FATAL = 1ULL << 63;
 
 enum {
@@ -49,6 +49,8 @@
   CI_N = 24
 };
 static_assert(CI_N == PINFO_CI_WORDS, "PushInfo holds a c1info copy");
+static_assert(offsetof(PushInfo, c1info) == offsetof(PushInfo, ctr) + CTR_ALLOC * 8,
+              "PushInfo mirrors the device's counter block + c1info block");
 
 __device__ __forceinline__ uint64_t key_hash(int64_t key) { return mix64((uint64_t)key ^ 0x6A09E667F3BCC908ULL); }
 
@@ -204,7 +206,7 @@
 void part_retry_trace_counts(const RetryPlan& r, bool listed, const std::vector<uint8_t>& host_fail, int64_t* nsub,
                              int64_t* fail_table, int64_t* fail_region);
 khip_status part_pass_commit(khip_agg* a, int pass, const RetryPlan& r, const int64_t* gate, const uint32_t* prn,
-                             const unsigned long long* closed_ctr, int64_t nT);
+                             const unsigned long long* closed_ctr, int64_t nT, bool pipeline);
 khip_status part_pass_failed(khip_agg* a, std::vector<uint8_t>* host_fail);
 void part_push_epilogue(khip_agg* a, int64_t closed_now, int64_t added, int64_t* tot);
 bool c1_eligible(khip_agg* a, int64_t n);
@@ -223,6 +225,7 @@
                               uint8_t* __restrict__ sel, int64_t* __restrict__ cnt,
                               unsigned long long* __restrict__ newcnt, const uint8_t* __restrict__ fail,
                               unsigned long long* __restrict__ out, unsigned long long* __restrict__ hcnt,
-                              unsigned long long* __restrict__ hnew);
-
-}
+                              unsigned long long* __restrict__ hnew, const unsigned long long* __restrict__ closed_n,
+                              const int64_t* __restrict__ stream_time);
+
+}
```

Measured after the change: 57.56 billion, median of 6. 1.03x the previous value.
